# deepomicslab/PALACE

Measured on AMD Instinct MI355X. Metric: contigs/sec eref+generate_graph+matching, 1M-contig synth, 1/2/4/8 GPU, higher is better.
Workload: dtype u32

## Files before the change

include/palace_hip.h:

```cpp
#ifndef PALACE_HIP_H
#define PALACE_HIP_H

#include <stddef.h>
#include <stdint.h>

#ifdef __cplusplus
extern "C" {
#endif

#define PALACE_OK 0
#define PALACE_EINVAL (-1)
#define PALACE_EHIP (-2)
#define PALACE_ENOMEM (-3)
#define PALACE_ESTATE (-4)

typedef struct palace_ctx palace_ctx;

const char *palace_last_error(void);
const char *palace_version(void);

int palace_ctx_create(int device, palace_ctx **out);
int palace_ctx_create_prio(int device, int high_priority, palace_ctx **out);
int palace_ctx_create_on_stream(int device, void *hip_stream, palace_ctx **out);
int palace_ctx_destroy(palace_ctx *ctx);
// ... 148 lines not shown
                            int64_t n_records_total, const palace_graph_params *prm, uint64_t *d_consumed,
                            palace_graph_edge *d_edges, int64_t edge_cap, int64_t *d_n_edges, int64_t *n_edges_out);

int palace_graph_score_border(palace_ctx *ctx, palace_graph_cand *d_cands, int64_t n_cands, int64_t n_border,
                              const palace_graph_params *prm);

int palace_graph_copy_numbers(palace_ctx *ctx, const uint64_t *d_consumed, const int32_t *d_tlen,
                              int32_t n_targets, double avg_depth, int32_t *d_cn);


int palace_bgzf_inflate(palace_ctx *ctx, const uint8_t *d_in, int64_t n_members, const int64_t *d_in_off, const int32_t *d_in_len,
                        const int64_t *d_out_off, const int32_t *d_out_len, uint8_t *d_out, int32_t *d_status);


int palace_bgzf_deflate(palace_ctx *ctx, const uint8_t *d_text, int64_t n_members, const int64_t *d_off, const int32_t *d_len,
                        const uint32_t *d_crc, uint8_t *d_slots, int32_t *d_member_len);

int palace_bgzf_deflate_lz(palace_ctx *ctx, const uint8_t *d_text, int64_t n_members, const int64_t *d_off, const int32_t *d_len,
                           const uint32_t *d_crc, uint8_t *d_slots, int32_t *d_member_len);

int palace_bgzf_compact(palace_ctx *ctx, const uint8_t *d_slots, int64_t n_members, const int32_t *d_member_len, uint8_t *d_file,
                        int64_t *d_member_off);


int palace_crc32_members(palace_ctx *ctx, const uint8_t *d_data, int64_t n_members, const int64_t *d_off, const int32_t *d_len,
                         uint32_t *d_crc);

typedef struct {
    int64_t line, reads, bases;
    int32_t open, error;
} palace_fastq_cursor;

size_t palace_fastq_scratch_bytes(int64_t max_window);
int palace_fastq_parse(palace_ctx *ctx, const uint8_t *d_text, int64_t n, int final_window, palace_fastq_cursor *d_cursor,
                       uint8_t *d_bases, int64_t bases_cap, int64_t *d_offsets, int64_t offsets_cap, void *d_scratch,
                       size_t scratch_bytes);


#define PALACE_DEPTH_TAIL_BYTES 4096

typedef struct {
    int64_t lines;
    uint64_t sum;
    int64_t bad_line;
    int64_t win_runs, win_name_bytes;
    int32_t tail_len, tail_buf;
    int32_t error, reserved0;
    int64_t reserved1;
    uint8_t tail[2][PALACE_DEPTH_TAIL_BYTES];
} palace_depth_cursor;

typedef struct {
    uint64_t sum, lines;
    uint32_t name_off, name_len;
} palace_depth_run;

size_t palace_depth_parse_scratch_bytes(int64_t max_window);
int palace_depth_parse(palace_ctx *ctx, const uint8_t *d_text, int64_t n, int final_window, palace_depth_cursor *d_cursor,
                       palace_depth_run *d_runs, int64_t runs_cap, uint8_t *d_names, int64_t names_cap, void *d_scratch,
                       size_t scratch_bytes);


typedef struct {
    int64_t stride, span, text_cap;
    int64_t check_guards;
} palace_gzip_params;

enum {
    PALACE_GZ_NONE = 0,
    PALACE_GZ_HEADER = 1,
    PALACE_GZ_DECODE = 2,
    PALACE_GZ_CHAIN_OPEN = 3,
    PALACE_GZ_NO_PROGRESS = 4,
    PALACE_GZ_TOO_BIG = 5,
    PALACE_GZ_TRUNCATED = 6,
    PALACE_GZ_CRC = 7,
    PALACE_GZ_ISIZE = 8,
    PALACE_GZ_TRAILING = 9,
    PALACE_GZ_SINK = 10,
    PALACE_GZ_MARKER = 11
};

typedef struct {
    int64_t chunks_found, chunks_accepted, false_hits, rounds, members, spans, batches, text_bytes;
    int32_t fallback, guards_bad;
    double ms_upload, ms_find, ms_size, ms_decode, ms_chain, ms_resolve, ms_crc, ms_sink;
} palace_gzip_stats;

typedef int (*palace_gzip_sink)(void *user, const uint8_t *d_text, int64_t n, int last);

int palace_gzip_inflate(palace_ctx *ctx, const uint8_t *file, int64_t size, const palace_gzip_params *prm, palace_gzip_sink sink,
                        void *user, palace_gzip_stats *stats);


int palace_depth_sum_covered(palace_ctx *ctx, int64_t n_segs, const int32_t *d_seg_tid, const int32_t *d_seg_pos,
                             const int32_t *d_seg_len, int32_t n_targets, const int32_t *d_tlen, const int64_t *d_tbase,
                             int64_t total_len, uint64_t *sum_out, uint64_t *covered_out);

int palace_depth_per_contig(palace_ctx *ctx, int64_t n_segs, const int32_t *d_seg_tid, const int32_t *d_seg_pos,
                            const int32_t *d_seg_len, int32_t n_targets, const int32_t *d_tlen, const int64_t *d_tbase,
                            int64_t total_len, uint64_t *sum_out, uint64_t *covered_out, uint64_t *d_contig_sum,
                            uint64_t *d_contig_covered);

typedef struct palace_depth_text palace_depth_text;
int palace_depth_text_create(palace_ctx *ctx, int64_t n_segs, const int32_t *d_seg_tid, const int32_t *d_seg_pos,
                             const int32_t *d_seg_len, int32_t n_targets, const int32_t *d_tlen, const int64_t *d_tbase,
                             int64_t total_len, const uint8_t *d_names, const int64_t *d_name_off, palace_depth_text **out,
                             uint64_t *text_bytes_out, uint64_t *lines_out, uint64_t *sum_out);
int palace_depth_text_destroy(palace_ctx *ctx, palace_depth_text *dt);
int palace_depth_text_emit(palace_ctx *ctx, const palace_depth_text *dt, uint64_t text_begin, uint64_t text_end, uint8_t *d_out);
int palace_depth_text_windows(palace_ctx *ctx, const palace_depth_text *dt, int64_t n_windows, const int64_t *d_win_beg,
                              const int64_t *d_win_end, uint64_t *d_text_beg, uint64_t *d_text_end, uint64_t *d_lines);


size_t palace_bam_walk_scratch_bytes(int64_t total, int64_t first, int64_t chunk);
int palace_bam_walk(palace_ctx *ctx, const uint8_t *d_stream, int64_t total, int64_t first, int32_t n_ref, int64_t chunk,
                    void *d_scratch, size_t scratch_bytes, int64_t *d_starts, int64_t cap, int64_t *n_records_out,
                    int64_t *stop_out, int64_t stats_out[4]);
int palace_bam_walk_starts(palace_ctx *ctx, const uint8_t *d_stream, int64_t total, int64_t first, int64_t chunk, const void *d_scratch,
                           size_t scratch_bytes, int64_t *d_starts, int64_t cap);

int palace_bam_match_segments(palace_ctx *ctx, const uint8_t *d_stream, int64_t total, const int64_t *d_starts, int64_t n_records,
                              int32_t n_ref, int32_t *d_seg_tid, int32_t *d_seg_pos, int32_t *d_seg_len, int64_t cap,
                              int64_t *n_segs_out);


int palace_bam_columns(palace_ctx *ctx, const uint8_t *d_stream, int64_t total, const int64_t *d_starts, int64_t n_records,
                       uint64_t key_seed, const palace_bam_cols *cols);
int palace_bam_name_keys(palace_ctx *ctx, const uint8_t *d_stream, int64_t total, const int64_t *d_starts, int64_t n_records,
                         uint64_t key_seed, uint64_t *d_qkey);
int palace_bam_names_differ(palace_ctx *ctx, const uint8_t *d_stream, int64_t total, const int64_t *d_starts, int64_t n_records,
                            const int64_t *d_pairs, int64_t n_pairs, int64_t *n_differ_out);

typedef struct palace_bam_names palace_bam_names;
int palace_bam_names_create(palace_ctx *ctx, const uint8_t *d_names, const int64_t *d_name_off, int32_t n_ref, palace_bam_names **out);
int palace_bam_names_destroy(palace_ctx *ctx, palace_bam_names *names);

int palace_bam_sa_items(palace_ctx *ctx, const uint8_t *d_stream, int64_t total, const int64_t *d_starts, int64_t n_records,
                        const palace_bam_names *names, int32_t *d_sa_off, palace_sa_item *d_items, int64_t cap, int64_t *n_items_out);


int palace_match_greedy(palace_ctx *ctx, int32_t n_vertices, int64_t n_arcs, const int32_t *d_src,
                        const int32_t *d_dst, const int64_t *d_out_off, const int32_t *d_out_arcs,
                        const int64_t *d_in_off, const int32_t *d_in_arcs, const uint8_t *d_alive,
                        int32_t *d_next, int32_t *d_prev, int32_t *d_next_arc, int32_t *rounds_out);

int palace_match_arcs_from_edges(const int32_t *cn, int32_t n_segs, const palace_graph_edge *edges, int64_t n_edges,
                                 int32_t min_count, int64_t *copies, int32_t *src, int32_t *dst, int64_t *weight,
                                 int64_t *n_arcs_out);

typedef struct palace_match_result palace_match_result;
int palace_match_set_option(palace_ctx *ctx, const char *name, int64_t value);
int palace_match_last_run(palace_ctx *ctx, int64_t info[4]);
int palace_match_decompose(palace_ctx *ctx, int32_t n_segs, const int64_t *copies, int64_t n_arcs,
                           const int32_t *src, const int32_t *dst, int32_t iterations, int32_t aggressive,
                           palace_match_result **out);
int palace_match_decompose_ex(palace_ctx *ctx, int32_t n_segs, const int64_t *copies, int64_t n_arcs,
                              const int32_t *src, const int32_t *dst, int32_t iterations, int32_t aggressive,
                              int32_t compact, palace_match_result **out);
const uint64_t *palace_match_result_bare(const palace_match_result *r);
int64_t palace_match_result_bare_count(const palace_match_result *r);
int64_t palace_match_result_count(const palace_match_result *r);
const int64_t *palace_match_result_offsets(const palace_match_result *r);
const int32_t *palace_match_result_verts(const palace_match_result *r);
const uint8_t *palace_match_result_kind(const palace_match_result *r);
const int32_t *palace_match_result_iter(const palace_match_result *r);
const int32_t *palace_match_result_open_at(const palace_match_result *r);
void palace_match_result_free(palace_match_result *r);


typedef struct {
    int32_t n_segs;
    int32_t min_count;
    const uint8_t *seed;
    const int32_t *tlen;
    const int32_t *rank;
    const int32_t *name_len;
    int64_t n_paths;
    const int64_t *path_off;
    const int32_t *path_tok;
} palace_stage04_inputs;

typedef struct palace_stage04 palace_stage04;
int palace_stage04_create(palace_ctx *ctx, const palace_stage04_inputs *in, palace_stage04 **out);
int palace_stage04_destroy(palace_ctx *ctx, palace_stage04 *s);

int palace_stage04_reserve(palace_ctx *ctx, palace_stage04 *s, int64_t edge_bound);

int palace_stage04_filter(palace_ctx *ctx, palace_stage04 *s, const palace_graph_edge *d_edges, const int64_t *d_n_edges,
                          int64_t edge_bound);
int palace_stage04_flags(palace_ctx *ctx, palace_stage04 *s, uint8_t *h_seg_flags, uint8_t *h_edge_flags, int64_t n_edges);
int palace_stage04_counts(palace_ctx *ctx, palace_stage04 *s, int64_t counts[8]);

int palace_stage04_match(palace_ctx *ctx, palace_stage04 *s, const palace_graph_edge *d_edges, const int32_t *d_cn,
                         int32_t iterations, int32_t aggressive, int32_t use_paths);
int palace_stage04_result(palace_ctx *ctx, palace_stage04 *s, palace_match_result **out, const int32_t **contig_of_out,
                          int64_t *n_segs_filtered_out);


#define PALACE_FASTA_TILE_BYTES 4096

typedef struct {
    int64_t name_off, name_len, seq_off, length, line_bases, line_width;
} palace_fasta_rec;

#define PALACE_FASTA_OK 0
#define PALACE_FASTA_ETEXT 1
#define PALACE_FASTA_ENAME 2
#define PALACE_FASTA_ERAGGED 3
#define PALACE_FASTA_EBLANK 4
#define PALACE_FASTA_EBYTE 5

typedef struct {
    int64_t n_records, bad_line;
    int32_t error, reserved;
} palace_fasta_status;

size_t palace_fasta_index_scratch_bytes(int64_t n);
int palace_fasta_index(palace_ctx *ctx, const uint8_t *d_text, int64_t n, palace_fasta_rec *d_recs, int64_t recs_cap, void *d_scratch,
                       size_t scratch_bytes, palace_fasta_status *status_out);

typedef struct palace_fasta_names palace_fasta_names;
int palace_fasta_names_create(palace_ctx *ctx, const uint8_t *d_text, const palace_fasta_rec *d_recs, int64_t n_records, uint8_t *d_dup,
                              palace_fasta_names **out);
int palace_fasta_names_destroy(palace_ctx *ctx, palace_fasta_names *names);

#define PALACE_PATH_NOTHING (-1)
#define PALACE_PATH_NOT_FOUND (-2)
#define PALACE_PATH_REVERSE 1
#define PALACE_PATH_SECOND_TRY 2

int palace_path_resolve(palace_ctx *ctx, const palace_fasta_names *names, const uint8_t *d_tok, const int64_t *d_tok_off, int64_t n_tok,
                        int32_t *d_code);

int palace_path_fasta_lengths(palace_ctx *ctx, const palace_fasta_rec *d_recs, const int32_t *d_code, int64_t n_tok, const int64_t *d_path_off,
                              int64_t n_paths, int64_t *d_tok_cum, int64_t *d_path_len);

int palace_path_fasta_write(palace_ctx *ctx, const uint8_t *d_text, const palace_fasta_rec *d_recs, const int32_t *d_code,
                            const int64_t *d_tok_cum, const int64_t *d_path_off, int64_t n_paths, const uint8_t *d_hdr,
                            const int64_t *d_hdr_off, const int64_t *d_path_out, int64_t lo, int64_t hi, uint8_t *d_out);


int palace_cycle_trim(palace_ctx *ctx, const int32_t *d_node, const int32_t *d_base, const int64_t *d_len, int64_t n_tok,
                      const int64_t *d_path_off, int64_t n_paths, const uint64_t *d_arcs, int64_t n_arcs, int64_t trim_threshold,
                      int64_t min_cycle_length, int32_t *d_first, int32_t *d_last);

int palace_final_fasta_lengths(palace_ctx *ctx, const palace_fasta_rec *d_recs, const int32_t *d_code, int64_t n_tok, const int64_t *d_path_off,
                               int64_t n_paths, int64_t sep_len, int64_t *d_tok_cum, int64_t *d_path_len);

int palace_final_fasta_write(palace_ctx *ctx, const uint8_t *d_text, const palace_fasta_rec *d_recs, const int32_t *d_code,
                             const int64_t *d_tok_cum, const int64_t *d_path_off, int64_t n_paths, const uint8_t *d_hdr,
                             const int64_t *d_hdr_off, const int64_t *d_path_out, int32_t sep_byte, int64_t lo, int64_t hi, uint8_t *d_out);


#define PALACE_BLAST_ECOLUMNS 1
#define PALACE_BLAST_ENAME 2
#define PALACE_BLAST_EIDENTITY 3
#define PALACE_BLAST_ELENGTH 4
#define PALACE_BLAST_EQUERY 5
#define PALACE_BLAST_EQEMPTY 6

int palace_blast_identity_cuts(double threshold, int64_t *cut);

int palace_blast_groups(palace_ctx *ctx, const uint8_t *d_text, const int64_t *d_line_start, int64_t n_lines, const palace_fasta_names *names,
                        int64_t n_records, double blast_ratio, const int64_t *cut, uint8_t *d_seg, int64_t *out);

#define PALACE_FILTERRES_REC_GENE 1
#define PALACE_FILTERRES_REC_S07 2
#define PALACE_FILTERRES_REC_S09 4
#define PALACE_FILTERRES_REC_BLAST 8
#define PALACE_FILTERRES_TAG_SELF 1
#define PALACE_FILTERRES_TAG_CYCLE 2
#define PALACE_FILTERRES_WRITE 1
#define PALACE_FILTERRES_PLAIN 2
#define PALACE_FILTERRES_SELFGENE 4
#define PALACE_FILTERRES_CYCLEGENE 8
#define PALACE_FILTERRES_CYCLESCORE 16
#define PALACE_FILTERRES_GENESCORE 32

int palace_filter_result_plan(palace_ctx *ctx, const int32_t *d_code, const int64_t *d_path_off, int64_t n_paths, const uint8_t *d_tag,
                              const palace_fasta_rec *d_recs, const uint8_t *d_rec_bits, uint8_t *d_class, int64_t *d_all_len);

int palace_paths_first_of_equal(palace_ctx *ctx, const int32_t *d_code, const int64_t *d_path_off, int64_t n_paths, const uint8_t *d_class,
                                int32_t hash_bits, uint8_t *d_first);


#define PALACE_FASTG_EPLUS 6
#define PALACE_FASTG_EHIGH 7
#define PALACE_FASTG_ECR 8
#define PALACE_FASTG_ENOLF 9
#define PALACE_FASTG_EEMPTY 10
#define PALACE_FASTG_ENONAME 11
#define PALACE_FASTG_EBASE 12

int palace_fastg_derive(palace_ctx *ctx, const uint8_t *d_text, int64_t n, const palace_fasta_rec *d_recs, int64_t n_records,
                        palace_fasta_rec *d_name_recs, uint8_t *d_primed, palace_fasta_status *status_out);

int palace_fastg_plan(palace_ctx *ctx, const palace_fasta_rec *d_name_recs, uint8_t *d_dup, int64_t n_records, int64_t *d_out_off,
                      palace_fasta_rec *d_out_recs, int64_t *n_kept_out, int64_t *out_bytes_out);

int palace_fastg_write(palace_ctx *ctx, const uint8_t *d_text, const palace_fasta_rec *d_name_recs, const uint8_t *d_primed,
                       const int64_t *d_out_off, int64_t n_records, int64_t lo, int64_t hi, uint8_t *d_out);

int palace_fai_rows_plan(palace_ctx *ctx, const palace_fasta_rec *d_recs, const uint8_t *d_skip, int64_t n_records, int64_t *d_row_off,
                         int64_t *bytes_out);
int palace_fai_rows_write(palace_ctx *ctx, const uint8_t *d_text, const palace_fasta_rec *d_recs, const uint8_t *d_skip, int64_t n_records,
// ... 164 lines not shown
```

palace_amd/capi.py:

```python
from __future__ import annotations

import ctypes as C
import os
import subprocess

import numpy as np

_HERE = os.path.dirname(os.path.abspath(__file__))
SO_PATH = os.environ.get("PALACE_HIP_SO") or os.path.join(_HERE, "libpalace_hip.so")
_LIB = None


class PalaceError(RuntimeError):
    pass


def build(force: bool = False) -> str:
    args = ["make", "-C", os.path.join(_HERE, "csrc")]
    if force:
        subprocess.run(args + ["clean"], check=True, stdout=subprocess.DEVNULL)
    subprocess.run(args, check=True, stdout=subprocess.DEVNULL)
    return SO_PATH


# ... 2 lines not shown
                ("both_order", C.c_int32), ("reserved", C.c_int32), ("max_span_frac", C.c_double)]

    @classmethod
    def default(cls):
        return cls(300, 0, 5, 1, 0, 0, 0.80)


class BamCols(C.Structure):
    _fields_ = [("n", C.c_int64)] + [(k, C.c_void_p) for k in
                                     ("tid", "pos", "mtid", "mpos", "nm", "ref_len", "read_len", "clip_s", "clip_e",
                                      "flag", "mapq", "qkey", "sa_off")]


class GzipParams(C.Structure):
    _fields_ = [("stride", C.c_int64), ("span", C.c_int64), ("text_cap", C.c_int64), ("check_guards", C.c_int64)]


class GzipStats(C.Structure):
    _fields_ = [(k, C.c_int64) for k in ("chunks_found", "chunks_accepted", "false_hits", "rounds", "members", "spans", "batches", "text_bytes")] + \
        [("fallback", C.c_int32), ("guards_bad", C.c_int32)] + \
        [(k, C.c_double) for k in ("ms_upload", "ms_find", "ms_size", "ms_decode", "ms_chain", "ms_resolve", "ms_crc", "ms_sink")]


GZIP_SINK = C.CFUNCTYPE(C.c_int, C.c_void_p, C.c_void_p, C.c_int64, C.c_int)


class Stage04Inputs(C.Structure):
    _fields_ = [("n_segs", C.c_int32), ("min_count", C.c_int32), ("seed", C.c_void_p), ("tlen", C.c_void_p), ("rank", C.c_void_p),
                ("name_len", C.c_void_p), ("n_paths", C.c_int64), ("path_off", C.c_void_p), ("path_tok", C.c_void_p)]


SA_ITEM_DTYPE = np.dtype([(k, np.int32) for k in ("tid2", "pos2", "mapq2", "nm2", "clip_s2", "clip_e2", "len2", "rev2")])
CAND_DTYPE = np.dtype([("ord", np.int64), ("qkey", np.uint64), ("left", np.int32), ("right", np.int32),
                       ("mtid", np.int32), ("ref_len", np.int32), ("dL", np.int32), ("dR", np.int32),
                       ("nmL", np.int32), ("nmR", np.int32), ("mapqL", np.int16), ("mapqR", np.int16),
                       ("kind", np.uint8), ("cls", np.uint8), ("found", np.uint8), ("in_fastg", np.uint8),
                       ("oL", np.uint8), ("oR", np.uint8), ("pad0", np.uint8), ("pad1", np.uint8), ("sa_index", np.int32)])
EDGE_DTYPE = np.dtype([("left", np.int32), ("right", np.int32), ("counts", np.uint32, 4), ("oL", np.uint8),
                       ("oR", np.uint8), ("pad", np.uint8, 6)])
FASTQ_CURSOR_DTYPE = np.dtype([("line", np.int64), ("reads", np.int64), ("bases", np.int64), ("open", np.int32), ("error", np.int32)])
DEPTH_CURSOR_DTYPE = np.dtype([("lines", np.int64), ("sum", np.uint64), ("bad_line", np.int64), ("win_runs", np.int64), ("win_name_bytes", np.int64),
                               ("tail_len", np.int32), ("tail_buf", np.int32), ("error", np.int32), ("reserved0", np.int32), ("reserved1", np.int64),
                               ("tail", np.uint8, (2, 4096))])
DEPTH_RUN_DTYPE = np.dtype([("sum", np.uint64), ("lines", np.uint64), ("name_off", np.uint32), ("name_len", np.uint32)])
assert DEPTH_CURSOR_DTYPE.itemsize == 64 + 8192 and DEPTH_RUN_DTYPE.itemsize == 24
FASTA_REC_DTYPE = np.dtype([(k, np.int64) for k in ("name_off", "name_len", "seq_off", "length", "line_bases", "line_width")])
FASTA_TILE_BYTES = 4096
FAIDX_REGION_DTYPE = np.dtype([(k, np.int64) for k in ("rec", "beg", "len")])
CONTIG_FEATURES, CONTIG_FSUMS, CONTIG_CHUNK_BASES = 12288, 64, 4096
CONTIG_INFO_DTYPE = np.dtype([("length", np.int64), ("bases", np.int64)])
PATH_NOTHING, PATH_NOT_FOUND, PATH_REVERSE, PATH_SECOND_TRY = -1, -2, 1, 2


class BaiStatus(C.Structure):
    _fields_ = [("n_bad", C.c_int64), ("first_bad", C.c_int64), ("first_unsorted", C.c_int64), ("n_no_coor", C.c_int64)]


SORT_TILE = 4096


class FastaStatus(C.Structure):
    _fields_ = [("n_records", C.c_int64), ("bad_line", C.c_int64), ("error", C.c_int32), ("reserved", C.c_int32)]


class ReadqcParams(C.Structure):
    _fields_ = [(k, C.c_int32) for k in ("qualified_quality", "unqualified_percent", "n_limit", "min_length", "no_trim", "no_quality_filter",
                                         "no_length_filter", "overlap_require", "diff_limit", "diff_pct", "diff_window", "reserved")]

    @classmethod
    def default(cls, **kw):
        p = cls(15, 40, 5, 15, 0, 0, 0, 30, 5, 20, 50, 0)
        for k, v in kw.items():
            assert hasattr(p, k), k
            setattr(p, k, int(v))
        return p


READQC_OUT = ("reads_before", "bases_before", "reads_after", "bases_after", "low_quality", "too_many_n", "too_short", "trimmed_reads", "trimmed_bases",
              "bytes_1", "bytes_2")
READQC_ISIZE_MAX = 512
READQC_CYCLE_TILE = 256

assert CAND_DTYPE.itemsize == 64 and EDGE_DTYPE.itemsize == 32 and SA_ITEM_DTYPE.itemsize == 32 and C.sizeof(ReadqcParams) == 48

_SIGS = {
    "palace_ctx_create": [C.c_int, C.POINTER(C.c_void_p)],
    "palace_ctx_create_prio": [C.c_int, C.c_int, C.POINTER(C.c_void_p)],
    "palace_ctx_create_on_stream": [C.c_int, C.c_void_p, C.POINTER(C.c_void_p)],
    "palace_ctx_destroy": [C.c_void_p],
    "palace_sync": [C.c_void_p],
    "palace_malloc": [C.c_void_p, C.c_size_t, C.POINTER(C.c_void_p)],
    "palace_free": [C.c_void_p, C.c_void_p],
    "palace_memset": [C.c_void_p, C.c_void_p, C.c_int, C.c_size_t],
    "palace_h2d": [C.c_void_p, C.c_void_p, C.c_void_p, C.c_size_t],
    "palace_d2h": [C.c_void_p, C.c_void_p, C.c_void_p, C.c_size_t],
    "palace_d2d": [C.c_void_p, C.c_void_p, C.c_void_p, C.c_size_t],
    "palace_host_alloc": [C.c_void_p, C.c_size_t, C.POINTER(C.c_void_p)],
    "palace_host_free": [C.c_void_p, C.c_void_p],
    "palace_d2h_async": [C.c_void_p, C.c_void_p, C.c_void_p, C.c_size_t],
    "palace_h2d_async": [C.c_void_p, C.c_void_p, C.c_void_p, C.c_size_t],
    "palace_mark_wait": [C.c_void_p, C.c_int],
    "palace_mark_wait_for": [C.c_void_p, C.c_int, C.c_double],
    "palace_wait_for_mark": [C.c_void_p, C.c_void_p, C.c_int],
    "palace_timer_begin": [C.c_void_p],
    "palace_timer_end": [C.c_void_p, C.POINTER(C.c_float)],
    "palace_mark": [C.c_void_p, C.c_int],
    "palace_mark_elapsed": [C.c_void_p, C.c_int, C.c_int, C.POINTER(C.c_float)],
    "palace_eref_set_coder": [C.c_void_p, C.c_void_p],
    "palace_eref_index_refs": [C.c_void_p, C.c_void_p, C.c_void_p, C.c_int64, C.c_void_p, C.c_void_p],
    "palace_eref_table_reset": [C.c_void_p],
    "palace_eref_reserve": [C.c_void_p, C.c_int64],
    "palace_eref_count_reads": [C.c_void_p, C.c_void_p, C.c_void_p, C.c_int64, C.c_void_p, C.c_int64],
    "palace_eref_pack_reads": [C.c_void_p, C.c_void_p, C.c_void_p, C.c_int64, C.c_void_p, C.c_int64, C.c_void_p, C.c_void_p, C.c_void_p],
    "palace_eref_count_reads_packed": [C.c_void_p, C.c_void_p, C.c_void_p, C.c_void_p, C.c_int64, C.c_int64],
    "palace_eref_set_count_mode": [C.c_void_p, C.c_int, C.c_int64],
    "palace_eref_set_key_buckets": [C.c_void_p, C.c_void_p],
    "palace_eref_set_option": [C.c_void_p, C.c_char_p, C.c_int64],
    "palace_eref_scan_refs": [C.c_void_p, C.c_void_p, C.c_void_p, C.c_int64, C.c_int64, C.c_int, C.c_int,
                              C.c_void_p],
    "palace_eref_probe_index_build": [C.c_void_p, C.c_void_p, C.c_void_p, C.c_int64, C.c_int64, C.POINTER(C.c_void_p)],
    "palace_eref_attach_probe_index": [C.c_void_p, C.c_void_p],
    "palace_eref_entry_layout": [C.c_void_p, C.POINTER(C.c_size_t), C.POINTER(C.c_size_t)],
    "palace_eref_entry_buffers_attach": [C.c_void_p, C.c_void_p, C.c_void_p, C.c_void_p],
    "palace_eref_entry_buffers": [C.c_void_p, C.POINTER(C.c_void_p), C.POINTER(C.c_void_p)],
    "palace_eref_entry_hits_from_counts": [C.c_void_p, C.c_void_p, C.c_void_p, C.c_int, C.c_size_t, C.c_size_t, C.c_size_t],
    "palace_eref_entry_hits_complete": [C.c_void_p, C.c_void_p, C.c_int64],
    "palace_eref_entry_counts_valid": [C.c_void_p, C.c_void_p],
    "palace_eref_probe_index_free": [C.c_void_p, C.c_void_p],
    "palace_eref_scan_refs_indexed": [C.c_void_p, C.c_void_p, C.c_void_p, C.c_void_p, C.c_int64, C.c_int64, C.c_int, C.c_int,
                                      C.c_void_p],
    "palace_eref_table_planes": [C.c_void_p, C.POINTER(C.c_void_p), C.POINTER(C.c_size_t)],
    "palace_eref_table_attach": [C.c_void_p, C.POINTER(C.c_void_p)],
    "palace_eref_table_invalidate": [C.c_void_p],
    "palace_eref_table_merge_slices": [C.c_void_p, C.c_void_p, C.c_int, C.c_size_t, C.c_size_t],
    "palace_eref_table_merge_slices_packed": [C.c_void_p, C.c_void_p, C.c_int, C.c_size_t, C.c_size_t],
    "palace_eref_table_pack_low": [C.c_void_p, C.c_void_p],
    "palace_eref_plane_pack": [C.c_void_p, C.c_void_p, C.c_void_p, C.c_void_p, C.c_int64, C.c_void_p],
    "palace_eref_plane_unpack": [C.c_void_p, C.c_void_p, C.c_void_p, C.c_void_p, C.c_int64, C.c_void_p],
    "palace_eref_table_lookup": [C.c_void_p, C.c_void_p, C.c_int64, C.c_void_p],
    "palace_eref_table_popcounts": [C.c_void_p, C.POINTER(C.c_uint64)],
    "palace_graph_classify": [C.c_void_p, C.POINTER(BamCols), C.c_void_p, C.c_int32, C.c_void_p, C.c_void_p,
                              C.c_void_p, C.c_int64, C.POINTER(GraphParams), C.c_int64, C.c_void_p, C.c_void_p,
                              C.c_int64, C.POINTER(C.c_int64)],
    "palace_depth_sum_covered": [C.c_void_p, C.c_int64, C.c_void_p, C.c_void_p, C.c_void_p, C.c_int32, C.c_void_p, C.c_void_p, C.c_int64,
                                 C.POINTER(C.c_uint64), C.POINTER(C.c_uint64)],
    "palace_depth_per_contig": [C.c_void_p, C.c_int64, C.c_void_p, C.c_void_p, C.c_void_p, C.c_int32, C.c_void_p, C.c_void_p, C.c_int64,
                                C.POINTER(C.c_uint64), C.POINTER(C.c_uint64), C.c_void_p, C.c_void_p],
    "palace_graph_copy_numbers": [C.c_void_p, C.c_void_p, C.c_void_p, C.c_int32, C.c_double, C.c_void_p],
    "palace_match_greedy": [C.c_void_p, C.c_int32, C.c_int64] + [C.c_void_p] * 10 + [C.POINTER(C.c_int32)],
    "palace_match_arcs_from_edges": [C.c_void_p, C.c_int32, C.c_void_p, C.c_int64, C.c_int32, C.c_void_p, C.c_void_p,
                                     C.c_void_p, C.c_void_p, C.POINTER(C.c_int64)],
    "palace_match_set_option": [C.c_void_p, C.c_char_p, C.c_int64],
    "palace_match_last_run": [C.c_void_p, C.POINTER(C.c_int64)],
    "palace_match_decompose":[C.c_void_p, C.c_int32, C.c_void_p, C.c_int64, C.c_void_p, C.c_void_p, C.c_int32,
                               C.c_int32, C.POINTER(C.c_void_p)],
    "palace_match_decompose_ex": [C.c_void_p, C.c_int32, C.c_void_p, C.c_int64, C.c_void_p, C.c_void_p, C.c_int32,
                                  C.c_int32, C.c_int32, C.POINTER(C.c_void_p)],
    "palace_graph_resolve": [C.c_void_p, C.c_void_p, C.c_int64, C.c_int64, C.POINTER(GraphParams), C.c_void_p,
                             C.c_void_p, C.c_int64, C.POINTER(C.c_int64)],
    "palace_graph_classify_ex": [C.c_void_p, C.POINTER(BamCols), C.c_void_p, C.c_int32, C.c_void_p, C.c_void_p,
                                 C.c_void_p, C.c_int64, C.POINTER(GraphParams), C.c_int64, C.c_void_p, C.c_void_p,
                                 C.c_int64, C.POINTER(C.c_int64), C.POINTER(C.c_int64)],
    "palace_graph_classify_ix": [C.c_void_p, C.POINTER(BamCols), C.c_void_p, C.c_int32, C.c_void_p, C.c_void_p,
                                 C.c_void_p, C.c_int64, C.c_void_p, C.POINTER(GraphParams), C.c_int64, C.c_void_p, C.c_void_p,
                                 C.c_int64, C.POINTER(C.c_int64), C.POINTER(C.c_int64)],
    "palace_graph_fastg_offsets": [C.c_void_p, C.c_void_p, C.c_int64, C.c_int32, C.c_void_p],
    "palace_bgzf_inflate": [C.c_void_p, C.c_void_p, C.c_int64, C.c_void_p, C.c_void_p, C.c_void_p, C.c_void_p, C.c_void_p, C.c_void_p],
    "palace_fastq_scratch_bytes": [C.c_int64],
    "palace_crc32_members": [C.c_void_p, C.c_void_p, C.c_int64, C.c_void_p, C.c_void_p, C.c_void_p],
    "palace_bgzf_deflate": [C.c_void_p, C.c_void_p, C.c_int64, C.c_void_p, C.c_void_p, C.c_void_p, C.c_void_p, C.c_void_p],
    "palace_bgzf_deflate_lz": [C.c_void_p, C.c_void_p, C.c_int64, C.c_void_p, C.c_void_p, C.c_void_p, C.c_void_p, C.c_void_p],
    "palace_bgzf_compact": [C.c_void_p, C.c_void_p, C.c_int64, C.c_void_p, C.c_void_p, C.c_void_p],
    "palace_depth_text_create": [C.c_void_p, C.c_int64, C.c_void_p, C.c_void_p, C.c_void_p, C.c_int32, C.c_void_p, C.c_void_p, C.c_int64,
                                 C.c_void_p, C.c_void_p, C.POINTER(C.c_void_p), C.POINTER(C.c_uint64), C.POINTER(C.c_uint64), C.POINTER(C.c_uint64)],
    "palace_depth_text_destroy": [C.c_void_p, C.c_void_p],
    "palace_depth_text_emit": [C.c_void_p, C.c_void_p, C.c_uint64, C.c_uint64, C.c_void_p],
    "palace_depth_text_windows": [C.c_void_p, C.c_void_p, C.c_int64, C.c_void_p, C.c_void_p, C.c_void_p, C.c_void_p, C.c_void_p],
    "palace_gzip_inflate": [C.c_void_p, C.c_void_p, C.c_int64, C.POINTER(GzipParams), GZIP_SINK, C.c_void_p, C.POINTER(GzipStats)],
    "palace_fastq_parse": [C.c_void_p, C.c_void_p, C.c_int64, C.c_int, C.c_void_p, C.c_void_p, C.c_int64, C.c_void_p, C.c_int64,
                           C.c_void_p, C.c_size_t],
    "palace_depth_parse_scratch_bytes": [C.c_int64],
    "palace_depth_parse": [C.c_void_p, C.c_void_p, C.c_int64, C.c_int, C.c_void_p, C.c_void_p, C.c_int64, C.c_void_p, C.c_int64,
                           C.c_void_p, C.c_size_t],
    "palace_graph_score_border": [C.c_void_p, C.c_void_p, C.c_int64, C.c_int64, C.POINTER(GraphParams)],
    "palace_graph_resolve_ex": [C.c_void_p, C.c_void_p, C.c_int64, C.c_int64, C.c_int64, C.POINTER(GraphParams), C.c_void_p,
                                C.c_void_p, C.c_int64, C.c_void_p, C.POINTER(C.c_int64)],
    "palace_bam_walk_scratch_bytes": [C.c_int64, C.c_int64, C.c_int64],
    "palace_bam_walk": [C.c_void_p, C.c_void_p, C.c_int64, C.c_int64, C.c_int32, C.c_int64, C.c_void_p, C.c_size_t, C.c_void_p, C.c_int64,
                        C.POINTER(C.c_int64), C.POINTER(C.c_int64), C.POINTER(C.c_int64)],
    "palace_bam_walk_starts": [C.c_void_p, C.c_void_p, C.c_int64, C.c_int64, C.c_int64, C.c_void_p, C.c_size_t, C.c_void_p, C.c_int64],
    "palace_bam_match_segments": [C.c_void_p, C.c_void_p, C.c_int64, C.c_void_p, C.c_int64, C.c_int32, C.c_void_p, C.c_void_p, C.c_void_p,
                                  C.c_int64, C.POINTER(C.c_int64)],
    "palace_bam_columns": [C.c_void_p, C.c_void_p, C.c_int64, C.c_void_p, C.c_int64, C.c_uint64, C.POINTER(BamCols)],
    "palace_bam_name_keys": [C.c_void_p, C.c_void_p, C.c_int64, C.c_void_p, C.c_int64, C.c_uint64, C.c_void_p],
    "palace_bam_names_differ": [C.c_void_p, C.c_void_p, C.c_int64, C.c_void_p, C.c_int64, C.c_void_p, C.c_int64, C.POINTER(C.c_int64)],
    "palace_bam_names_create": [C.c_void_p, C.c_void_p, C.c_void_p, C.c_int32, C.POINTER(C.c_void_p)],
    "palace_bam_names_destroy": [C.c_void_p, C.c_void_p],
    "palace_bam_sa_items": [C.c_void_p, C.c_void_p, C.c_int64, C.c_void_p, C.c_int64, C.c_void_p, C.c_void_p, C.c_void_p, C.c_int64,
                            C.POINTER(C.c_int64)],
    "palace_stage04_create": [C.c_void_p, C.POINTER(Stage04Inputs), C.POINTER(C.c_void_p)],
    "palace_stage04_destroy": [C.c_void_p, C.c_void_p],
    "palace_stage04_reserve": [C.c_void_p, C.c_void_p, C.c_int64],
    "palace_stage04_filter": [C.c_void_p, C.c_void_p, C.c_void_p, C.c_void_p, C.c_int64],
    "palace_stage04_flags": [C.c_void_p, C.c_void_p, C.c_void_p, C.c_void_p, C.c_int64],
    "palace_stage04_counts": [C.c_void_p, C.c_void_p, C.POINTER(C.c_int64)],
    "palace_stage04_match": [C.c_void_p, C.c_void_p, C.c_void_p, C.c_void_p, C.c_int32, C.c_int32, C.c_int32],
    "palace_stage04_result": [C.c_void_p, C.c_void_p, C.POINTER(C.c_void_p), C.POINTER(C.c_void_p), C.POINTER(C.c_int64)],
    "palace_fasta_index_scratch_bytes": [C.c_int64],
    "palace_fasta_index": [C.c_void_p, C.c_void_p, C.c_int64, C.c_void_p, C.c_int64, C.c_void_p, C.c_size_t, C.POINTER(FastaStatus)],
    "palace_fasta_names_create": [C.c_void_p, C.c_void_p, C.c_void_p, C.c_int64, C.c_void_p, C.POINTER(C.c_void_p)],
    "palace_fasta_names_destroy": [C.c_void_p, C.c_void_p],
    "palace_path_resolve": [C.c_void_p, C.c_void_p, C.c_void_p, C.c_void_p, C.c_int64, C.c_void_p],
    "palace_path_fasta_lengths": [C.c_void_p, C.c_void_p, C.c_void_p, C.c_int64, C.c_void_p, C.c_int64, C.c_void_p, C.c_void_p],
    "palace_fastg_derive": [C.c_void_p, C.c_void_p, C.c_int64, C.c_void_p, C.c_int64, C.c_void_p, C.c_void_p, C.POINTER(FastaStatus)],
    "palace_fastg_plan": [C.c_void_p, C.c_void_p, C.c_void_p, C.c_int64, C.c_void_p, C.c_void_p, C.POINTER(C.c_int64), C.POINTER(C.c_int64)],
    "palace_fastg_write": [C.c_void_p, C.c_void_p, C.c_void_p, C.c_void_p, C.c_void_p, C.c_int64, C.c_int64, C.c_int64, C.c_void_p],
    "palace_fai_rows_plan": [C.c_void_p, C.c_void_p, C.c_void_p, C.c_int64, C.c_void_p, C.POINTER(C.c_int64)],
    "palace_fai_rows_write": [C.c_void_p, C.c_void_p, C.c_void_p, C.c_void_p, C.c_int64, C.c_void_p, C.c_void_p],
    "palace_faidx_resolve": [C.c_void_p, C.c_void_p, C.c_void_p, C.c_void_p, C.c_void_p, C.c_int64, C.c_void_p],
    "palace_faidx_plan": [C.c_void_p, C.c_void_p, C.c_int64, C.c_void_p, C.c_int64, C.c_int, C.c_void_p, C.POINTER(C.c_int64), C.POINTER(C.c_int64)],
    "palace_faidx_write": [C.c_void_p, C.c_void_p, C.c_void_p, C.c_void_p, C.c_int64, C.c_void_p, C.c_void_p, C.c_void_p, C.c_int64, C.c_int, C.c_int64,
                           C.c_int64, C.c_void_p],
    "palace_path_fasta_write": [C.c_void_p, C.c_void_p, C.c_void_p, C.c_void_p, C.c_void_p, C.c_void_p, C.c_int64, C.c_void_p, C.c_void_p,
                                C.c_void_p, C.c_int64, C.c_int64, C.c_void_p],
    "palace_cycle_trim": [C.c_void_p, C.c_void_p, C.c_void_p, C.c_void_p, C.c_int64, C.c_void_p, C.c_int64, C.c_void_p, C.c_int64, C.c_int64, C.c_int64,
                          C.c_void_p, C.c_void_p],
    "palace_final_fasta_lengths": [C.c_void_p, C.c_void_p, C.c_void_p, C.c_int64, C.c_void_p, C.c_int64, C.c_int64, C.c_void_p, C.c_void_p],
    "palace_final_fasta_write": [C.c_void_p, C.c_void_p, C.c_void_p, C.c_void_p, C.c_void_p, C.c_void_p, C.c_int64, C.c_void_p, C.c_void_p,
                                 C.c_void_p, C.c_int32, C.c_int64, C.c_int64, C.c_void_p],
    "palace_blast_identity_cuts": [C.c_double, C.POINTER(C.c_int64)],
    "palace_blast_groups": [C.c_void_p, C.c_void_p, C.c_void_p, C.c_int64, C.c_void_p, C.c_int64, C.c_double, C.POINTER(C.c_int64), C.c_void_p,
                            C.POINTER(C.c_int64)],
    "palace_filter_result_plan": [C.c_void_p, C.c_void_p, C.c_void_p, C.c_int64, C.c_void_p, C.c_void_p, C.c_void_p, C.c_void_p, C.c_void_p],
    "palace_paths_first_of_equal": [C.c_void_p, C.c_void_p, C.c_void_p, C.c_int64, C.c_void_p, C.c_int32, C.c_void_p],
    "palace_bam_sort_keys": [C.c_void_p, C.c_void_p, C.c_int64, C.c_void_p, C.c_int64, C.c_int32, C.c_void_p, C.POINTER(C.c_int64), C.POINTER(C.c_int64)],
    "palace_sort_u64_scratch_bytes": [C.c_int64],
    "palace_sort_u64": [C.c_void_p, C.c_void_p, C.c_void_p, C.c_int64, C.c_int32, C.c_void_p, C.c_size_t],
    "palace_bam_gather_plan": [C.c_void_p, C.c_void_p, C.c_void_p, C.c_void_p, C.c_int64, C.c_int64, C.c_void_p, C.c_void_p, C.POINTER(C.c_int64)],
    "palace_bam_gather_write": [C.c_void_p, C.c_void_p, C.c_void_p, C.c_void_p, C.c_void_p, C.c_int64, C.c_int64, C.c_void_p],
    "palace_bai_records": [C.c_void_p, C.c_void_p, C.c_void_p, C.c_int64, C.c_int32, C.c_void_p, C.c_void_p, C.c_void_p, C.c_void_p, C.c_void_p,
                           C.POINTER(BaiStatus)],
    "palace_bai_chunks": [C.c_void_p, C.c_void_p, C.c_void_p, C.c_void_p, C.c_void_p, C.c_int64, C.c_int32, C.c_void_p, C.c_void_p, C.c_void_p, C.c_void_p,
                          C.c_int64, C.POINTER(C.c_int64)],
    "palace_bai_linear": [C.c_void_p, C.c_void_p, C.c_void_p, C.c_void_p, C.c_void_p, C.c_void_p, C.c_void_p, C.c_int64, C.c_int32, C.c_void_p, C.c_void_p,
                          C.c_void_p, C.c_int64, C.c_void_p],
    "palace_bgzf_voffsets": [C.c_void_p, C.c_void_p, C.c_int64, C.c_void_p, C.c_void_p, C.c_int64, C.c_void_p],
    "palace_sam_scratch_bytes": [C.c_int64],
    "palace_sam_lines": [C.c_void_p, C.c_void_p, C.c_int64, C.c_void_p, C.c_size_t, C.c_void_p, C.c_int64, C.POINTER(C.c_int64)],
    "palace_sam_plan": [C.c_void_p, C.c_void_p, C.c_void_p, C.c_int64, C.c_int64, C.c_void_p, C.c_uint32, C.c_int64, C.c_void_p, C.c_void_p, C.c_void_p,
                        C.POINTER(C.c_int64)],
    "palace_sam_encode": [C.c_void_p, C.c_void_p, C.c_void_p, C.c_int64, C.c_void_p, C.c_void_p, C.c_void_p, C.c_void_p, C.c_void_p, C.c_void_p],
    "palace_fastq_records": [C.c_void_p, C.c_void_p, C.c_void_p, C.c_int64, C.c_void_p, C.POINTER(C.c_int64)],
    "palace_readqc_plan": [C.c_void_p, C.c_void_p, C.c_void_p, C.c_void_p, C.c_void_p, C.c_int64, C.POINTER(ReadqcParams), C.c_void_p, C.c_void_p, C.c_void_p,
                           C.c_void_p, C.POINTER(C.c_int64)],
    "palace_readqc_write": [C.c_void_p, C.c_void_p, C.c_void_p, C.c_void_p, C.c_void_p, C.c_int64, C.c_int64, C.c_int64, C.c_void_p],
    "palace_readqc_plan_ex": [C.c_void_p, C.c_void_p, C.c_void_p, C.c_void_p, C.c_void_p, C.c_int64, C.POINTER(ReadqcParams), C.c_void_p, C.c_void_p, C.c_void_p,
                              C.c_void_p, C.c_void_p, C.POINTER(C.c_int64)],
    "palace_readqc_insert_sizes": [C.c_void_p, C.c_void_p, C.c_void_p, C.c_void_p, C.c_int64, C.POINTER(ReadqcParams), C.c_void_p],
    "palace_readqc_cycle_stats": [C.c_void_p, C.c_void_p, C.c_void_p, C.c_int64, C.c_void_p, C.c_int32, C.c_void_p],
    "palace_contig_features_scratch_bytes": [C.c_int64, C.c_int64],
    "palace_contig_features": [C.c_void_p, C.c_void_p, C.c_int64, C.c_void_p, C.c_int64, C.c_int64, C.c_void_p, C.c_void_p, C.c_void_p, C.c_void_p,
                               C.c_void_p, C.c_size_t],
}


def declared_symbols():
    import re
    text = open(os.path.join(_HERE, "..", "include", "palace_hip.h")).read()
    text = re.sub(r"/\*.*?\*/", "", text, flags=re.S)
    return sorted(set(re.findall(r"\b(palace_[a-z0-9_]+)\s*\(", text)))


def lib() -> C.CDLL:
    global _LIB
    if _LIB is None:
        if not os.path.exists(SO_PATH):
            raise PalaceError(f"{SO_PATH} is missing: run `python -c 'import __graft_entry__ as g; g.build()'` "
                              "(hipcc --offload-arch=gfx950). There is no CPU fallback.")
        _LIB = C.CDLL(SO_PATH)
        _LIB.palace_last_error.restype = C.c_char_p
        _LIB.palace_version.restype = C.c_char_p
        _LIB.palace_stream.restype = C.c_void_p
        _LIB.palace_stream.argtypes = [C.c_void_p]
        _LIB.palace_eref_packed_bytes.restype = C.c_size_t
        _LIB.palace_eref_packed_bytes.argtypes = [C.c_int64]
        for nm, rt in (("count", C.c_int64), ("bare_count", C.c_int64), ("bare", C.POINTER(C.c_uint64)), ("offsets", C.POINTER(C.c_int64)), ("verts", C.POINTER(C.c_int32)),
                       ("kind", C.POINTER(C.c_uint8)), ("iter", C.POINTER(C.c_int32)), ("open_at", C.POINTER(C.c_int32))):
            fn = getattr(_LIB, "palace_match_result_" + nm)
            fn.argtypes = [C.c_void_p]
            fn.restype = rt
        _LIB.palace_match_result_free.argtypes = [C.c_void_p]
        _LIB.palace_match_result_free.restype = None
        for name, sig in _SIGS.items():
            fn = getattr(_LIB, name)
            fn.argtypes = sig
            fn.restype = C.c_int
        _LIB.palace_fastq_scratch_bytes.restype = C.c_size_t
        _LIB.palace_bam_walk_scratch_bytes.restype = C.c_size_t
        _LIB.palace_depth_parse_scratch_bytes.restype = C.c_size_t
        _LIB.palace_fasta_index_scratch_bytes.restype = C.c_size_t
        _LIB.palace_sort_u64_scratch_bytes.restype = C.c_size_t
        _LIB.palace_sam_scratch_bytes.restype = C.c_size_t
        _LIB.palace_contig_features_scratch_bytes.restype = C.c_size_t
    return _LIB


# ... 955 lines not shown

    def close(self):
        for b in self.bufs:
            b.free()
        self.bufs = []


BAM_COLUMNS = (("tid", np.int32), ("pos", np.int32), ("mtid", np.int32), ("mpos", np.int32), ("nm", np.int32), ("ref_len", np.int32),
               ("read_len", np.int32), ("clip_s", np.int32), ("clip_e", np.int32), ("flag", np.uint16), ("mapq", np.uint8), ("qkey", np.uint64))


def bam_decode(ctx: Ctx, stream: bytes, starts, names, key_seed: int = 1):
    stream = bytes(stream)
    st = np.ascontiguousarray(starts, dtype=np.int64)
    n = len(st)
    blob = b"".join(names)
    off = np.zeros(len(names) + 1, np.int64)
    off[1:] = np.cumsum([len(x) for x in names])
    bufs = [ctx.upload(np.frombuffer(stream, dtype=np.uint8) if stream else np.zeros(1, np.uint8)), ctx.upload(st if n else np.zeros(1, np.int64)),
            ctx.upload(np.frombuffer(blob, dtype=np.uint8) if blob else np.zeros(1, np.uint8)), ctx.upload(off)]
    d_stream, d_st, d_blob, d_off = bufs
    table = C.c_void_p()
    try:
        col = {k: ctx.empty(max(1, n), dt) for k, dt in BAM_COLUMNS}
        col["sa_off"] = ctx.empty(n + 1, np.int32)
        bufs += list(col.values())
        cols = BamCols(n, **{k: b.ptr for k, b in col.items()})
        _check(lib().palace_bam_columns(ctx.h, d_stream.ptr, len(stream), d_st.ptr, n, key_seed, C.byref(cols)), "palace_bam_columns")
        _check(lib().palace_bam_names_create(ctx.h, d_blob.ptr, d_off.ptr, len(names), C.byref(table)), "palace_bam_names_create")
        cnt = C.c_int64()
        _check(lib().palace_bam_sa_items(ctx.h, d_stream.ptr, len(stream), d_st.ptr, n, table, None, None, 0, C.byref(cnt)), "palace_bam_sa_items")
        want = cnt.value
        d_items = ctx.empty(max(1, want), SA_ITEM_DTYPE)
        bufs.append(d_items)
        _check(lib().palace_bam_sa_items(ctx.h, d_stream.ptr, len(stream), d_st.ptr, n, table, col["sa_off"].ptr, d_items.ptr, want, C.byref(cnt)),
               "palace_bam_sa_items")
        assert cnt.value == want
        out = {k: b.to_host()[:n + 1 if k == "sa_off" else n].copy() for k, b in col.items()}
        return out, d_items.to_host()[:want].copy()
    finally:
        if table:
            lib().palace_bam_names_destroy(ctx.h, table)
        for b in bufs:
            b.free()


def bam_name_keys(ctx: Ctx, stream: bytes, starts, key_seed: int):
    stream = bytes(stream)
    st = np.ascontiguousarray(starts, dtype=np.int64)
    bufs = [ctx.upload(np.frombuffer(stream, dtype=np.uint8)), ctx.upload(st), ctx.empty(max(1, len(st)), np.uint64)]
    try:
        _check(lib().palace_bam_name_keys(ctx.h, bufs[0].ptr, len(stream), bufs[1].ptr, len(st), key_seed, bufs[2].ptr), "palace_bam_name_keys")
        return bufs[2].to_host()[:len(st)].copy()
    finally:
        for b in bufs:
            b.free()


def bam_names_differ(ctx: Ctx, stream: bytes, starts, pairs) -> int:
    stream = bytes(stream)
    st = np.ascontiguousarray(starts, dtype=np.int64)
    pr = np.ascontiguousarray(pairs, dtype=np.int64).reshape(-1, 2)
    bufs = [ctx.upload(np.frombuffer(stream, dtype=np.uint8)), ctx.upload(st), ctx.upload(pr if len(pr) else np.zeros((1, 2), np.int64))]
    n = C.c_int64()
    try:
        _check(lib().palace_bam_names_differ(ctx.h, bufs[0].ptr, len(stream), bufs[1].ptr, len(st), bufs[2].ptr, len(pr), C.byref(n)),
               "palace_bam_names_differ")
        return int(n.value)
    finally:
        for b in bufs:
            b.free()


_ARC_BUFFERS = {}


def match_arcs_from_edges(cn: np.ndarray, edges: np.ndarray, min_count: int = 5, reuse: bool = False):
    cn = np.ascontiguousarray(cn, dtype=np.int32)
    e = np.ascontiguousarray(edges, dtype=EDGE_DTYPE)
    key = (len(cn), len(e))
    if reuse and key in _ARC_BUFFERS:
        copies, src, dst, w = _ARC_BUFFERS[key]
    else:
        copies = np.empty(len(cn), np.int64)
        src = np.empty(2 * len(e), np.int32); dst = np.empty(2 * len(e), np.int32); w = np.empty(2 * len(e), np.int64)
        if reuse:
            _ARC_BUFFERS.clear()
            _ARC_BUFFERS[key] = (copies, src, dst, w)
    n = C.c_int64()
    _check(lib().palace_match_arcs_from_edges(cn.ctypes.data, len(cn), e.ctypes.data, len(e), min_count, copies.ctypes.data,
                                              src.ctypes.data, dst.ctypes.data, w.ctypes.data, C.byref(n)),
           "palace_match_arcs_from_edges")
    return copies, src[:n.value], dst[:n.value], w[:n.value]


class MatchResult:

    def __init__(self, handle):
        L = lib()
        self._h = handle
        n = self.n = L.palace_match_result_count(handle)
        self.off = np.ctypeslib.as_array(L.palace_match_result_offsets(handle), shape=(n + 1,))
        nv = int(self.off[-1])
        self.verts = np.ctypeslib.as_array(L.palace_match_result_verts(handle), shape=(max(nv, 1),))[:nv]
        mk = lambda f, dt: (np.ctypeslib.as_array(f(handle), shape=(max(n, 1),))[:n] if n else np.zeros(0, dt))
        self.kind = mk(L.palace_match_result_kind, np.uint8)
        self.iter = mk(L.palace_match_result_iter, np.int32)
        self.open_at = mk(L.palace_match_result_open_at, np.int32)

    def free(self):
        if self._h is not None:
            self.off = self.verts = self.kind = self.iter = self.open_at = None
            lib().palace_match_result_free(self._h)
            self._h = None

    def __enter__(self):
        return self

    def __exit__(self, *exc):
        self.free()


def match_decompose_views(ctx: "Ctx", copies: np.ndarray, src: np.ndarray, dst: np.ndarray, iterations: int = 10,
                          aggressive: bool = False, compact: bool = False) -> MatchResult:
    cp = np.ascontiguousarray(copies, dtype=np.int64)
    s = np.ascontiguousarray(src, dtype=np.int32)
    d = np.ascontiguousarray(dst, dtype=np.int32)
    res = C.c_void_p()
    _check(lib().palace_match_decompose_ex(ctx.h, len(cp), cp.ctypes.data, len(s), s.ctypes.data, d.ctypes.data,
                                           iterations, int(aggressive), int(compact), C.byref(res)), "palace_match_decompose")
    r = MatchResult(res)
    if compact:
        r.n_bare = int(lib().palace_match_result_bare_count(res))
        words = (len(cp) + 63) // 64
        r.bare = np.ctypeslib.as_array(lib().palace_match_result_bare(res), shape=(max(1, words),))[:words]
    return r


def match_decompose(ctx: "Ctx", copies: np.ndarray, src: np.ndarray, dst: np.ndarray, iterations: int = 10,
                    aggressive: bool = False):
    with match_decompose_views(ctx, copies, src, dst, iterations, aggressive) as r:
        return r.off.copy(), r.verts.copy(), r.kind.copy(), r.iter.copy(), r.open_at.copy()


MATCH_KEYS_POSITION, MATCH_KEYS_TWO_WORDS, MATCH_KEYS_ONE_WORD = 0, 1, 2


def match_last_run(ctx: "Ctx") -> dict:
    info = (C.c_int64 * 4)()
    _check(lib().palace_match_last_run(ctx.h, info), "palace_match_last_run")
    return dict(key_mode=int(info[0]), checked_rerun=bool(info[1]), rounds=int(info[2]), iterations=int(info[3]))


def match_greedy(ctx: "Ctx", n_vertices: int, src, dst, alive=None):
    s = np.ascontiguousarray(src, dtype=np.int32)
    d = np.ascontiguousarray(dst, dtype=np.int32)
    al = np.ones(n_vertices, np.uint8) if alive is None else np.ascontiguousarray(alive, dtype=np.uint8)
    assert len(s) == len(d) and len(al) == n_vertices
    assert not len(s) or (0 <= min(s.min(), d.min()) and max(s.max(), d.max()) < n_vertices)

    def csr(ends):
        off = np.zeros(n_vertices + 1, np.int64)
        np.cumsum(np.bincount(ends, minlength=n_vertices), out=off[1:])
        return off, np.argsort(ends, kind="stable").astype(np.int32)

    (out_off, out_arcs), (in_off, in_arcs) = csr(s), csr(d)
    bufs = [ctx.upload(a) for a in (s, d, out_off, out_arcs, in_off, in_arcs, al)]
    outs = [ctx.empty(max(1, n_vertices), np.int32) for _ in range(3)]
    rounds = C.c_int32()
    try:
        _check(lib().palace_match_greedy(ctx.h, n_vertices, len(s), *(b.ptr for b in bufs), *(o.ptr for o in outs), C.byref(rounds)),
               "palace_match_greedy")
        nxt, prv, arc = (o.to_host()[:n_vertices] for o in outs)
    finally:
        for b in bufs + outs:
            b.free()
    return nxt, prv, arc, rounds.value


class Stage04:
    COUNT_NAMES = ("edges", "juncs", "kept_pass2", "kept_pass3_more", "segs_selected", "segs_rescued", "arcs", "segs_filtered")

    def __init__(self, ctx: "Ctx", seed, tlen, rank, name_len, path_off, path_tok, min_count: int = 5):
        self.ctx = ctx
        self._keep = [np.ascontiguousarray(seed, np.uint8), np.ascontiguousarray(tlen, np.int32), np.ascontiguousarray(rank, np.int32),
                      np.ascontiguousarray(name_len, np.int32), np.ascontiguousarray(path_off, np.int64),
                      np.ascontiguousarray(path_tok, np.int32)]
        sd, tl, rk, nl, po, pt = self._keep
        assert len(sd) == len(tl) == len(rk) == len(nl) and len(po) >= 1
        inp = Stage04Inputs(len(sd), min_count, sd.ctypes.data, tl.ctypes.data, rk.ctypes.data, nl.ctypes.data, len(po) - 1,
                            po.ctypes.data, pt.ctypes.data if len(pt) else None)
        h = C.c_void_p()
        _check(lib().palace_stage04_create(ctx.h, C.byref(inp), C.byref(h)), "palace_stage04_create")
        self.h, self.n_segs = h, len(sd)

    def filter(self, d_edges_ptr: int, d_n_edges_ptr: int, edge_bound: int):
        _check(lib().palace_stage04_filter(self.ctx.h, self.h, d_edges_ptr, d_n_edges_ptr, edge_bound), "palace_stage04_filter")

    def counts(self) -> dict:
        out = (C.c_int64 * 8)()
        _check(lib().palace_stage04_counts(self.ctx.h, self.h, out), "palace_stage04_counts")
        return dict(zip(self.COUNT_NAMES, (int(v) for v in out)))

    def flags(self, n_edges: int):
        seg = np.zeros(self.n_segs, np.uint8)
        edge = np.zeros(n_edges, np.uint8)
        _check(lib().palace_stage04_flags(self.ctx.h, self.h, seg.ctypes.data, edge.ctypes.data if n_edges else None, n_edges),
               "palace_stage04_flags")
        return seg, edge

    def match(self, d_edges_ptr: int, d_cn_ptr: int, iterations: int = 10, aggressive: bool = False, use_paths: bool = True):
        _check(lib().palace_stage04_match(self.ctx.h, self.h, d_edges_ptr, d_cn_ptr, iterations, int(aggressive), int(use_paths)), "palace_stage04_match")

    def result(self):
        res, cof, n = C.c_void_p(), C.c_void_p(), C.c_int64()
        _check(lib().palace_stage04_result(self.ctx.h, self.h, C.byref(res), C.byref(cof), C.byref(n)), "palace_stage04_result")
        r = MatchResult(res)
        r.n_bare = int(lib().palace_match_result_bare_count(res))
        words = (n.value + 63) // 64
        r.bare = np.ctypeslib.as_array(lib().palace_match_result_bare(res), shape=(max(1, words),))[:words]
        contig_of = np.ctypeslib.as_array(C.cast(cof, C.POINTER(C.c_int32)), shape=(max(1, n.value),))[: n.value]
        return r, contig_of

    def close(self):
        if self.h:
            lib().palace_stage04_destroy(self.ctx.h, self.h)
            self.h = None


def window_minimums(hit_ratio: float, perfect_ratio: float):
    w = np.float32(500)
    return int(w * np.float32(hit_ratio)), int(w * np.float32(perfect_ratio))


def fasta_index(ctx: Ctx, text: bytes, recs_cap: int | None = None):
    a = np.frombuffer(text, dtype=np.uint8)
    d_text = ctx.upload(a)
    d_scratch = DevBuf(ctx, max(int(lib().palace_fasta_index_scratch_bytes(len(a))), 1))
    st = FastaStatus()
    if recs_cap is None:
        _check(lib().palace_fasta_index(ctx.h, d_text.ptr, len(a), None, 0, d_scratch.ptr, d_scratch.nbytes, C.byref(st)), "palace_fasta_index")
        recs_cap = int(st.n_records)
    d_recs = ctx.empty((max(recs_cap, 1),), FASTA_REC_DTYPE)
    _check(lib().palace_fasta_index(ctx.h, d_text.ptr, len(a), d_recs.ptr, recs_cap, d_scratch.ptr, d_scratch.nbytes, C.byref(st)), "palace_fasta_index")
    d_scratch.free()
    recs = d_recs.to_host()[:int(st.n_records)] if int(st.n_records) <= recs_cap else None
    return st, recs, d_text, d_recs


def fasta_index_at(ctx: Ctx, text_ptr: int, n: int, recs_ptr, recs_cap: int, scratch_ptr: int, scratch_bytes: int) -> FastaStatus:
    st = FastaStatus()
    _check(lib().palace_fasta_index(ctx.h, text_ptr, n, recs_ptr, recs_cap, scratch_ptr, scratch_bytes, C.byref(st)), "palace_fasta_index")
    return st


def contig_features_enqueue(ctx: Ctx, text_ptr: int, n: int, recs_ptr: int, r0: int, r1: int, feat_ptr: int, fsum_ptr: int, info_ptr, bad_ptr: int,
                            scratch_ptr: int, scratch_bytes: int):
    _check(lib().palace_contig_features(ctx.h, text_ptr, n, recs_ptr, r0, r1, feat_ptr, fsum_ptr, info_ptr, bad_ptr, scratch_ptr, scratch_bytes),
           "palace_contig_features")


def contig_features(ctx: Ctx, text: bytes, r0: int = 0, r1: int | None = None, guard_rows: int = 1, repeat: int = 1):
    st, recs, d_text, d_recs = fasta_index(ctx, text)
    if st.error:
        return st, recs, None, None, None, None
    n_rec = int(st.n_records)
    r1 = n_rec if r1 is None else r1
    rows = r1 - r0
    outs = []
    for width, dtype in ((CONTIG_FEATURES, np.float32), (CONTIG_FSUMS, np.float32), (1, CONTIG_INFO_DTYPE)):
        outs.append(ctx.upload(np.full((rows + 2 * guard_rows) * width * np.dtype(dtype).itemsize, 0xA5, np.uint8)))
    d_bad = ctx.upload(np.array([12345], np.int64))
    need = int(lib().palace_contig_features_scratch_bytes(len(text), rows))
    d_scratch = DevBuf(ctx, max(need, 1))
    at = [b.ptr + guard_rows * w * isz for b, w, isz in zip(outs, (CONTIG_FEATURES, CONTIG_FSUMS, 1), (4, 4, 16))]
    for _ in range(repeat):
        contig_features_enqueue(ctx, d_text.ptr, len(text), d_recs.ptr, r0, r1, at[0], at[1], at[2], d_bad.ptr, d_scratch.ptr, need)
    ctx.sync()
    got = []
    for b, width, dtype in zip(outs, (CONTIG_FEATURES, CONTIG_FSUMS, 1), (np.float32, np.float32, CONTIG_INFO_DTYPE)):
        raw = b.to_host()
        g = guard_rows * width * np.dtype(dtype).itemsize
        if not ((raw[:g] == 0xA5).all() and (raw[len(raw) - g:] == 0xA5).all()):
            raise PalaceError("palace_contig_features wrote outside its rows")
        got.append(raw[g:len(raw) - g].view(dtype).reshape(rows, width) if width > 1 else raw[g:len(raw) - g].view(dtype))
    bad = int(d_bad.to_host()[0])
    for b in outs + [d_bad, d_scratch, d_text, d_recs]:
        b.free()
    return st, recs, got[0], got[1], got[2], bad


class PathFasta:

    def __init__(self, ctx: Ctx, text: bytes):
        self.ctx = ctx
        self.status, self.recs, self.d_text, self.d_recs = fasta_index(ctx, text)
        assert self.status.error == 0, (self.status.error, self.status.bad_line)
        self.n = int(self.status.n_records)
        self.d_dup = ctx.empty((max(self.n, 1),), np.uint8)
        self.names = C.c_void_p()
        _check(lib().palace_fasta_names_create(ctx.h, self.d_text.ptr, self.d_recs.ptr, self.n, self.d_dup.ptr, C.byref(self.names)), "palace_fasta_names_create")

    def duplicates(self) -> np.ndarray:
        return self.d_dup.to_host()[:self.n]

    def resolve(self, tokens):
# ... 312 lines not shown
```

palace_amd/csrc/common.hpp:

```cpp
#pragma once
#include <hip/hip_runtime.h>
#include <cstdarg>
#include <cstdint>
#include <cstdio>
#include <cstring>
#include <vector>

#include "../../include/palace_hip.h"
#include "eref_table_state.hpp"

namespace palace {

void set_error(const char *fmt, ...);

#define PALACE_HIP_TRY(expr)                                                                    \
    do {                                                                                        \
        hipError_t e__ = (expr);                                                                \
        if (e__ != hipSuccess) {                                                                \
            palace::set_error("%s failed: %s (%s:%d)", #expr, hipGetErrorString(e__), __FILE__, \
                              __LINE__);                                                        \
            return PALACE_EHIP;                                                                 \
        }                                                                                       \
    } while (0)

#define PALACE_REQUIRE_AS(name, cond, msg)                         \
    do {                                                           \
        if (!(cond)) {                                             \
            palace::set_error("%s: %s", name, msg);                \
            return PALACE_EINVAL;                                  \
        }                                                          \
    } while (0)
#define PALACE_REQUIRE(cond, msg) PALACE_REQUIRE_AS(__func__, cond, msg)

constexpr int kWave = 64;
constexpr int kCUs = 256;
constexpr size_t kPlaneBytes = 1ull << 29;
constexpr size_t kPlaneWords = 1ull << 27;

struct CoderMasks {
    uint32_t m[3][3];
};

inline size_t align256(size_t b) { return (b + 255) & ~static_cast<size_t>(255); }

struct Workspace {
    void *ptr = nullptr;
    size_t bytes = 0;
};

}

namespace palace {
struct MatchScratch;
void free_match_scratch(MatchScratch *m);
}

struct palace_ctx {
    int device = 0;
    hipStream_t stream = nullptr;
    bool owns_stream = true;
    hipEvent_t ev0 = nullptr, ev1 = nullptr;
    uint32_t key_buckets[4] = {~0u, ~0u, ~0u, ~0u};
    std::vector<hipEvent_t> marks;
    bool coder_set = false;
    palace::CoderMasks masks{};
    uint32_t *plane[3] = {nullptr, nullptr, nullptr};
    bool planes_external = false;
    palace::TableState table;
    bool want_final = false;
    const struct palace_eref_probe_index *probe_ix = nullptr;
    int probe_all_sets = 0;
    int64_t scan_ref_lo = 0, scan_ref_hi = 0;
    int count_mode = 0;
    int64_t bin_cap_override = 0;
    int64_t slab_override = 0;
    palace::Workspace ws;
    bool ws_grown = false;
    palace::Workspace pin;
    palace::MatchScratch *match_scratch = nullptr;
    int64_t graph_border = -1;
    const void *graph_border_cands = nullptr;
    int64_t graph_border_n = -1;
    int match_grid = 0;
    bool match_two_word_keys = false;
    int match_iters = 0;
    int64_t match_last[4] = {-1, 0, 0, 0};
    uint64_t *d_small = nullptr;
};

namespace palace {
int ensure_workspace(palace_ctx *ctx, size_t bytes);
int ensure_pinned(palace_ctx *ctx, size_t bytes);
int ensure_table(palace_ctx *ctx);
}
```

palace_amd/csrc/decomp.hip:

```cpp
#include "decomp.hpp"

#include <algorithm>

namespace palace {

namespace {

constexpr uint64_t kNoKey = ~0ull;
constexpr uint64_t kClosed = 0;
constexpr int kStampShift = 42;
constexpr int kPackedShift = 52, kPackedStamps = 1 << (64 - kPackedShift);
constexpr uint64_t kLenMask = (1ull << 40) - 1;


__device__ __forceinline__ uint64_t wave_incl_scan(uint64_t v, int lane)
{
#pragma unroll
    for (int d = 1; d < 64; d <<= 1) {
        const uint64_t u = __shfl_up(v, d);
        if (lane >= d) v += u;
    }
    return v;
}

constexpr int kMaxWaves = 16;

__device__ void scan_partials_body(const uint64_t *__restrict__ in, int64_t n, uint64_t *__restrict__ partials, int blk, int nblk)
{
    __shared__ uint64_t part[kMaxWaves];
    const int64_t chunk = (n + nblk - 1) / nblk;
    const int64_t a = min(n, static_cast<int64_t>(blk) * chunk), e = min(n, a + chunk);
    uint64_t s = 0;
    for (int64_t i = a + threadIdx.x; i < e; i += blockDim.x) s += in[i];
    const int lane = threadIdx.x & 63, waves = static_cast<int>(blockDim.x >> 6);
    s = wave_incl_scan(s, lane);
    if (lane == 63) part[threadIdx.x >> 6] = s;
    __syncthreads();
    if (threadIdx.x == 0) {
        uint64_t t = 0;
        for (int w = 0; w < waves; w++) t += part[w];
        partials[blk] = t;
    }
    __syncthreads();
}

__device__ void scan_prefix_body(uint64_t *__restrict__ partials, int n_parts, uint64_t *__restrict__ total)
{
    __shared__ uint64_t part[kMaxWaves];
    const int lane = threadIdx.x & 63, wv = threadIdx.x >> 6;
    const uint64_t x = static_cast<int>(threadIdx.x) < n_parts ? partials[threadIdx.x] : 0;
    const uint64_t incl = wave_incl_scan(x, lane);
    if (lane == 63) part[wv] = incl;
    __syncthreads();
    uint64_t before = 0;
    for (int w = 0; w < wv; w++) before += part[w];
    if (static_cast<int>(threadIdx.x) < n_parts) partials[threadIdx.x] = before + incl - x;
    if (threadIdx.x == blockDim.x - 1) *total = before + incl;
    __syncthreads();
}

__device__ void scan_apply_body(const uint64_t *__restrict__ in, uint64_t *__restrict__ out, int64_t n, const uint64_t *__restrict__ partials,
                                int blk, int nblk)
{
    __shared__ uint64_t part[kMaxWaves];
    const int64_t chunk = (n + nblk - 1) / nblk;
    const int64_t a = min(n, static_cast<int64_t>(blk) * chunk), e = min(n, a + chunk);
    const int lane = threadIdx.x & 63, wv = threadIdx.x >> 6, waves = static_cast<int>(blockDim.x >> 6);
    uint64_t carry = partials[blk];
    for (int64_t base = a; base < e; base += blockDim.x) {
        const int64_t i = base + threadIdx.x;
        const uint64_t x = i < e ? in[i] : 0;
        const uint64_t incl = wave_incl_scan(x, lane);
        if (lane == 63) part[wv] = incl;
        __syncthreads();
        uint64_t before = 0, all = 0;
        for (int w = 0; w < waves; w++) { if (w < wv) before += part[w]; all += part[w]; }
        if (i < e) out[i] = carry + before + incl - x;
        carry += all;
        __syncthreads();
    }
}

__global__ __launch_bounds__(kDecompBlock) void scan_partials_kernel(const uint64_t *__restrict__ in, const int32_t *__restrict__ n_dev,
                                                                     uint64_t *__restrict__ partials)
{
    scan_partials_body(in, *n_dev, partials, static_cast<int>(blockIdx.x), static_cast<int>(gridDim.x));
}
__global__ __launch_bounds__(kDecompBlock) void scan_prefix_kernel(uint64_t *__restrict__ partials, int n_parts, uint64_t *__restrict__ total)
{
    scan_prefix_body(partials, n_parts, total);
}
__global__ __launch_bounds__(kDecompBlock) void scan_apply_kernel(const uint64_t *__restrict__ in, uint64_t *__restrict__ out,
                                                                  const int32_t *__restrict__ n_dev, const uint64_t *__restrict__ partials)
{
    scan_apply_body(in, out, *n_dev, partials, static_cast<int>(blockIdx.x), static_cast<int>(gridDim.x));
}

struct Span { int tid, n; };
__device__ __forceinline__ Span whole_grid() { return Span{static_cast<int>(blockIdx.x * blockDim.x + threadIdx.x), static_cast<int>(gridDim.x * blockDim.x)}; }

__device__ void ph_init(const DecompBufs &b, Span T, int64_t comp_cap, int64_t vert_cap, int n_flags, int allow_packed)
{
    DecompState *st = b.st;
    const int V = st->V;
    for (int i = T.tid; i < V; i += T.n) { b.bo_hi[i] = kNoKey; b.bi_hi[i] = kNoKey; b.on_path[i] = 0; }
    for (int i = T.tid; i < n_flags; i += T.n) b.changed[i] = 0;
    if (T.tid == 0) {
        st->n_comp = 0; st->n_vert = 0; st->comp_cap = comp_cap; st->vert_cap = vert_cap;
        st->unsettled = 0; st->overflow = 0; st->bad = 0; st->dead = 0; st->scan_total = 0; st->alive_after = 0;
        st->packed = (allow_packed && b.kc && b.pack_bad && *b.pack_bad == 0) ? 1u : 0u;
        if (comp_cap >= 0) b.o_off[0] = 0;
    }
}

__device__ void ph_round_begin(const DecompBufs &b, Span T, int reset_left)
{
    const int V = b.st->V;
    if (!reset_left && b.st->dead) return;
    if (T.tid == 0) { b.st->alive_after = 0; if (reset_left) b.st->dead = 0; }
    const int64_t E = b.st->E;
    for (int64_t e = T.tid; e < E; e += T.n) b.done[e] = 0;
    const bool packed = b.st->packed != 0;
    for (int i = T.tid; i < V; i += T.n) {
        const int s = i >> 1;
        const int64_t l = reset_left ? 1 : b.left[s];
        if (reset_left && !(i & 1)) b.left[s] = 1;
        b.alive[i] = l > 0;
        b.next[i] = -1; b.prev[i] = -1;
        b.bo_hi[i] = b.bi_hi[i] = l > 0 ? kNoKey : kClosed;
        if (!packed) { b.bo_lo[i] = kNoKey; b.bo_lo[V + i] = kNoKey; b.bi_lo[i] = kNoKey; b.bi_lo[V + i] = kNoKey; }
        b.len_a[i] = 0;
    }
}

struct IterArgs {
    uint64_t stamp;
    uint64_t stamp_p;
    int parity;
    int prev_flag, flag;
    int unique_hi;
};


__device__ void ph_propose_hi(const DecompBufs &b, Span T, const IterArgs &a)
{
    if (b.st->dead) return;
    if (a.prev_flag >= 0 && !b.changed[a.prev_flag]) return;
    const int64_t E = b.st->E;
    const int V = b.st->V;
    const int other = (a.parity ^ 1) * V;
    const bool packed = b.st->packed != 0;
    for (int64_t e = T.tid; e < E; e += T.n) {
        if (b.done[e]) continue;
        const int u = b.src[e], v = b.dst[e];
        if (b.bi_hi[v] == kClosed) { b.done[e] = 1; continue; }
        const uint64_t k = packed ? (a.stamp_p | b.kc[e]) : (a.stamp | b.khi[e]);
        if (atomicMin(reinterpret_cast<unsigned long long *>(&b.bo_hi[u]), static_cast<unsigned long long>(k)) == kClosed) { b.done[e] = 1; continue; }
        atomicMin(reinterpret_cast<unsigned long long *>(&b.bi_hi[v]), static_cast<unsigned long long>(k));
        if (!a.unique_hi && !packed) { b.bo_lo[other + u] = kNoKey; b.bi_lo[other + v] = kNoKey; }
    }
}

__device__ void ph_propose_lo(const DecompBufs &b, Span T, const IterArgs &a)
{
    if (b.st->dead) return;
    if (a.prev_flag >= 0 && !b.changed[a.prev_flag]) return;
    if (b.st->packed) return;
    const int64_t E = b.st->E;
    const int mine = a.parity * b.st->V;
    for (int64_t e = T.tid; e < E; e += T.n) {
        if (b.done[e]) continue;
        const int u = b.src[e], v = b.dst[e];
        const uint64_t k = a.stamp | b.khi[e], lo = b.klo[e];
        if (b.bo_hi[u] == k) atomicMin(reinterpret_cast<unsigned long long *>(&b.bo_lo[mine + u]), static_cast<unsigned long long>(lo));
        if (b.bi_hi[v] == k) atomicMin(reinterpret_cast<unsigned long long *>(&b.bi_lo[mine + v]), static_cast<unsigned long long>(lo));
    }
}

__device__ void ph_commit_flag(const DecompBufs &b, Span T, const IterArgs &a, volatile unsigned int *took);
__device__ void ph_commit(const DecompBufs &b, Span T, const IterArgs &a)
{
    if (b.st->dead) return;
    if (a.prev_flag >= 0 && !b.changed[a.prev_flag]) return;
    ph_commit_flag(b, T, a, b.changed + a.flag);
}
__device__ void ph_commit_flag(const DecompBufs &b, Span T, const IterArgs &a, volatile unsigned int *took)
{
    bool any = false;
    const int64_t E = b.st->E;
    const int mine = a.parity * b.st->V;
    const bool packed = b.st->packed != 0;
    for (int64_t e = T.tid; e < E; e += T.n) {
        if (b.done[e]) continue;
        const int u = b.src[e], v = b.dst[e];
        const uint64_t k = packed ? (a.stamp_p | b.kc[e]) : (a.stamp | b.khi[e]);
        if (b.bo_hi[u] != k || b.bi_hi[v] != k) continue;
        const uint64_t lo = b.klo[e];
        if (!a.unique_hi && !packed && (b.bo_lo[mine + u] != lo || b.bi_lo[mine + v] != lo)) continue;
        b.next[u] = v; b.prev[v] = u;
        b.nhi[u] = b.khi[e]; b.nlo[u] = lo;
        b.bo_hi[u] = kClosed; b.bi_hi[v] = kClosed;
        b.done[e] = 1;
        any = true;
    }
    if (__syncthreads_or(any) && threadIdx.x == 0) *took = 1u;
}

__device__ void ph_heads(const DecompBufs &b, Span T, int round, int last_flag)
{
    DecompState *st = b.st;
    if (st->dead) return;
    if (T.tid == 0 && last_flag >= 0 && b.changed[last_flag]) st->unsettled = 1;
    const int V = st->V;
    for (int v = T.tid; v < V; v += T.n) {
        if (!b.alive[v] || b.prev[v] >= 0) continue;
        int len = 0, last = v;
        int64_t least = b.left[v >> 1];
        for (int x = v; x >= 0; x = b.next[x]) {
            b.on_path[x] = round + 1;
            last = x;
            len++;
            least = min(least, b.left[x >> 1]);
        }
        const int twin_first = last ^ 1;
        if (v > twin_first) continue;
        const int64_t uses = twin_first == v ? 2 : 1;
        b.len_a[v] = (1ull << 40) | static_cast<uint64_t>(len);
        b.pay[v] = max(static_cast<int64_t>(1), least / uses);
        b.kind[v] = 0;
        b.open_at[v] = 0;
    }
}

__device__ void ph_cycles(const DecompBufs &b, Span T, int round)
{
    const int V = b.st->V;
    if (b.st->dead) return;
    for (int v = T.tid; v < V; v += T.n) {
        if (!b.alive[v] || b.on_path[v] == round + 1) continue;
        int len = 1, twin_least = v ^ 1, worst = 0;
        uint64_t whi = b.nhi[v], wlo = b.nlo[v];
        int64_t least = b.left[v >> 1];
        bool first = true;
        for (int x = b.next[v]; x != v; x = b.next[x]) {
            if (x < v) { first = false; break; }
            twin_least = min(twin_least, x ^ 1);
            const uint64_t hi = b.nhi[x], lo = b.nlo[x];
            if (hi > whi || (hi == whi && lo > wlo)) { whi = hi; wlo = lo; worst = len; }
            least = min(least, b.left[x >> 1]);
            len++;
        }
        if (!first || v > twin_least) continue;
        const int64_t uses = twin_least == v ? 2 : 1;
        b.len_a[v] = (1ull << 40) | static_cast<uint64_t>(len);
        b.pay[v] = max(static_cast<int64_t>(1), least / uses);
        b.kind[v] = 1;
        b.open_at[v] = (worst + 1) % len;
    }
}

__device__ void ph_emit(const DecompBufs &b, Span T, int round, int64_t c0, int64_t v0)
{
    DecompState *st = b.st;
    const int V = st->V;
    if (st->dead) return;
    int64_t alive = 0;
    for (int v = T.tid; v < V; v += T.n) {
        const uint64_t la = b.len_a[v];
        if (!la) continue;
        const int64_t len = static_cast<int64_t>(la & kLenMask);
        const uint64_t p = b.pos[v];
        const int64_t c = c0 + static_cast<int64_t>(p >> 40), at = v0 + static_cast<int64_t>(p & kLenMask);
        const int64_t pay = b.pay[v];
        const bool room = c < st->comp_cap && at + len <= st->vert_cap;
        if (!room) st->overflow = 1;
        else { b.o_off[c] = at; b.o_kind[c] = b.kind[v]; b.o_iter[c] = round; b.o_open[c] = b.open_at[v]; }
        int x = v;
        int64_t still = 0;
        for (int64_t k = 0; k < len; k++) {
            if (room) b.o_verts[at + k] = 2 * b.orig[x >> 1] + (x & 1);
            const int64_t l = b.left[x >> 1];
            b.left[x >> 1] = max(static_cast<int64_t>(0), l - pay);
            still += l - pay > 0;
            x = b.next[x];
        }
        alive += still;
    }
    __shared__ unsigned long long wg_alive;
    if (threadIdx.x == 0) wg_alive = 0;
    __syncthreads();
    if (alive) atomicAdd(&wg_alive, static_cast<unsigned long long>(alive));
    __syncthreads();
    if (threadIdx.x == 0 && wg_alive) atomicAdd(reinterpret_cast<unsigned long long *>(&st->alive_after), wg_alive);
}


__global__ void dec_init_kernel(DecompBufs b, int64_t comp_cap, int64_t vert_cap, int n_flags, int allow_packed) { ph_init(b, whole_grid(), comp_cap, vert_cap, n_flags, allow_packed); }
__global__ void dec_round_begin_kernel(DecompBufs b, int reset_left) { ph_round_begin(b, whole_grid(), reset_left); }
__global__ void dec_propose_hi_kernel(DecompBufs b, IterArgs a) { ph_propose_hi(b, whole_grid(), a); }
__global__ void dec_propose_lo_kernel(DecompBufs b, IterArgs a) { ph_propose_lo(b, whole_grid(), a); }
__global__ void dec_commit_kernel(DecompBufs b, IterArgs a) { ph_commit(b, whole_grid(), a); }
__global__ void dec_heads_kernel(DecompBufs b, int round, int last_flag) { ph_heads(b, whole_grid(), round, last_flag); }
__global__ void dec_cycles_kernel(DecompBufs b, int round) { ph_cycles(b, whole_grid(), round); }
__global__ void dec_emit_kernel(DecompBufs b, int round) { ph_emit(b, whole_grid(), round, b.st->n_comp, b.st->n_vert); }

__global__ void dec_round_end_kernel(DecompBufs b)
{
    DecompState *st = b.st;
    if (blockIdx.x || threadIdx.x || st->dead) return;
    st->dead = st->alive_after == 0;
    st->n_comp += static_cast<int64_t>(st->scan_total >> 40);
    st->n_vert += static_cast<int64_t>(st->scan_total & kLenMask);
    if (st->n_comp <= st->comp_cap) b.o_off[st->n_comp] = st->n_vert;
}

size_t up256(size_t v) { return (v + 255) / 256 * 256; }

struct Carver {
    char *base;
    size_t used = 0;
    template <class T>
    T *take(size_t n)
    {
        T *p = base ? reinterpret_cast<T *>(base + used) : nullptr;
        used += up256(std::max<size_t>(1, n) * sizeof(T));
        return p;
    }
};

size_t carve_all(DecompBufs &b, char *base, int64_t s_cap, int64_t e_cap, int64_t comp_cap, int64_t vert_cap, int rounds, int iters)
{
    Carver c{base};
    const size_t S = static_cast<size_t>(std::max<int64_t>(1, s_cap)), V = 2 * S, E = static_cast<size_t>(std::max<int64_t>(1, e_cap));
    b.st = c.take<DecompState>(1);
    b.src = c.take<int32_t>(E); b.dst = c.take<int32_t>(E);
    b.khi = c.take<uint64_t>(E); b.klo = c.take<uint64_t>(E);
    b.done = c.take<uint8_t>(E);
    b.kc = c.take<uint64_t>(E);
    b.left = c.take<int64_t>(S); b.orig = c.take<int32_t>(S);
    b.next = c.take<int32_t>(V); b.prev = c.take<int32_t>(V); b.on_path = c.take<int32_t>(V); b.open_at = c.take<int32_t>(V);
    b.nhi = c.take<uint64_t>(V); b.nlo = c.take<uint64_t>(V);
    b.bo_hi = c.take<uint64_t>(V); b.bi_hi = c.take<uint64_t>(V);
    b.bo_lo = c.take<uint64_t>(2 * V); b.bi_lo = c.take<uint64_t>(2 * V);
    b.len_a = c.take<uint64_t>(V); b.pos = c.take<uint64_t>(V);
    b.pay = c.take<int64_t>(V);
    b.alive = c.take<uint8_t>(V); b.kind = c.take<uint8_t>(V);
    b.partials = c.take<uint64_t>(kDecompGrid + 1);
    b.changed = c.take<uint32_t>(static_cast<size_t>(rounds) * static_cast<size_t>(iters));
    b.o_off = c.take<int64_t>(static_cast<size_t>(comp_cap) + 1);
    b.o_verts = c.take<int32_t>(static_cast<size_t>(vert_cap));
    b.o_iter = c.take<int32_t>(static_cast<size_t>(comp_cap));
    b.o_open = c.take<int32_t>(static_cast<size_t>(comp_cap));
    b.o_kind = c.take<uint8_t>(static_cast<size_t>(comp_cap));
    return c.used;
}

}

size_t decomp_bytes(int64_t s_cap, int64_t e_cap, int64_t comp_cap, int64_t vert_cap, int rounds, int iters)
{
    DecompBufs tmp;
    return carve_all(tmp, nullptr, s_cap, e_cap, comp_cap, vert_cap, rounds, iters);
}

void decomp_carve(DecompBufs &b, char *base, int64_t s_cap, int64_t e_cap, int64_t comp_cap, int64_t vert_cap, int rounds, int iters)
{
    carve_all(b, base, s_cap, e_cap, comp_cap, vert_cap, rounds, iters);
}

int scan_u64(palace_ctx *ctx, const uint64_t *in, uint64_t *out, const int32_t *n_dev, uint64_t *partials, uint64_t *total_dev)
{
    hipLaunchKernelGGL(scan_partials_kernel, dim3(kDecompGrid), dim3(kDecompBlock), 0, ctx->stream, in, n_dev, partials);
    hipLaunchKernelGGL(scan_prefix_kernel, dim3(1), dim3(kDecompBlock), 0, ctx->stream, partials, kDecompGrid, total_dev);
    hipLaunchKernelGGL(scan_apply_kernel, dim3(kDecompGrid), dim3(kDecompBlock), 0, ctx->stream, in, out, n_dev, partials);
    PALACE_HIP_TRY(hipGetLastError());
    return PALACE_OK;
}

namespace {

const dim3 kBlock(kDecompBlock);
constexpr int kWideGridDefault = 2048;
inline dim3 wide_grid(const palace_ctx *ctx) { return dim3(ctx->match_grid > 0 ? ctx->match_grid : kWideGridDefault); }

void enqueue_iterations(palace_ctx *ctx, const DecompBufs &b, int first, int n, uint64_t *count, int flag0, bool unique_hi)
{
    for (int k = 0; k < n; k++) {
        IterArgs a{((1ull << 21) - 1 - *count) << kStampShift, static_cast<uint64_t>((kPackedStamps - 1 - *count) & (kPackedStamps - 1)) << kPackedShift,
                   (first + k) & 1, k ? flag0 + k - 1 : -1, flag0 + k, unique_hi ? 1 : 0};
        (*count)++;
        hipLaunchKernelGGL(dec_propose_hi_kernel, wide_grid(ctx), kBlock, 0, ctx->stream, b, a);
        if (!unique_hi) hipLaunchKernelGGL(dec_propose_lo_kernel, wide_grid(ctx), kBlock, 0, ctx->stream, b, a);
        hipLaunchKernelGGL(dec_commit_kernel, wide_grid(ctx), kBlock, 0, ctx->stream, b, a);
    }
}

int enqueue_read_off(palace_ctx *ctx, const DecompBufs &b, int round, int last_flag)
{
    hipLaunchKernelGGL(dec_heads_kernel, wide_grid(ctx), kBlock, 0, ctx->stream, b, round, last_flag);
    hipLaunchKernelGGL(dec_cycles_kernel, wide_grid(ctx), kBlock, 0, ctx->stream, b, round);
    int rc = scan_u64(ctx, b.len_a, b.pos, &b.st->V, b.partials, &b.st->scan_total);
    if (rc) return rc;
    hipLaunchKernelGGL(dec_emit_kernel, wide_grid(ctx), kBlock, 0, ctx->stream, b, round);
    hipLaunchKernelGGL(dec_round_end_kernel, dim3(1), dim3(64), 0, ctx->stream, b);
    PALACE_HIP_TRY(hipGetLastError());
    return PALACE_OK;
}

}

int decomp_begin(palace_ctx *ctx, const DecompBufs &b, int rounds, int64_t comp_cap, int64_t vert_cap)
{
    PALACE_REQUIRE(rounds >= 1 && rounds <= kMaxRounds, "round count out of range");
    static_assert(kDecompGrid <= kDecompBlock, "scan_prefix_kernel scans the block sums with one workgroup");
    const int allow_packed = !ctx->match_two_word_keys && static_cast<int64_t>(rounds) * kMaxIters < kPackedStamps ? 1 : 0;
    hipLaunchKernelGGL(dec_init_kernel, wide_grid(ctx), kBlock, 0, ctx->stream, b, comp_cap, vert_cap, rounds * kMaxIters, allow_packed);
    PALACE_HIP_TRY(hipGetLastError());
    return PALACE_OK;
}

int decomp_rounds(palace_ctx *ctx, const DecompBufs &b, int t0, int t1, int rounds, int aggressive, int iters, bool unique_hi,
                  uint64_t *count)
{
    PALACE_REQUIRE(0 <= t0 && t0 <= t1 && t1 <= rounds && rounds <= kMaxRounds && iters >= 1 && iters <= kMaxIters, "round / iteration count out of range");
    for (int t = t0; t < t1; t++) {
        hipLaunchKernelGGL(dec_round_begin_kernel, wide_grid(ctx), kBlock, 0, ctx->stream, b, (aggressive && t == rounds - 1) ? 1 : 0);
        enqueue_iterations(ctx, b, 0, iters, count, t * kMaxIters, unique_hi);
        int rc = enqueue_read_off(ctx, b, t, t * kMaxIters + iters - 1);
        if (rc) return rc;
    }
    PALACE_HIP_TRY(hipGetLastError());
    return PALACE_OK;
}

int decomp_run_checked(palace_ctx *ctx, const DecompBufs &b, int rounds, int aggressive, bool unique_hi, int64_t comp_cap,
                       int64_t vert_cap, int64_t max_iterations, uint64_t *iterations_out)
{
    PALACE_REQUIRE(rounds >= 1 && rounds <= kMaxRounds, "round count out of range");
    constexpr int kBatch = 16;
    hipLaunchKernelGGL(dec_init_kernel, wide_grid(ctx), kBlock, 0, ctx->stream, b, comp_cap, vert_cap, kBatch, 0);
    uint64_t count = 0;
    for (int t = 0; t < rounds; t++) {
        hipLaunchKernelGGL(dec_round_begin_kernel, wide_grid(ctx), kBlock, 0, ctx->stream, b, (aggressive && t == rounds - 1) ? 1 : 0);
        for (int first = 0;; first += kBatch) {
            PALACE_HIP_TRY(hipMemsetAsync(b.changed, 0, kBatch * sizeof(uint32_t), ctx->stream));
            enqueue_iterations(ctx, b, first, kBatch, &count, 0, unique_hi);
            uint32_t last = 0;
            PALACE_HIP_TRY(hipMemcpyAsync(&last, b.changed + kBatch - 1, sizeof last, hipMemcpyDeviceToHost, ctx->stream));
            PALACE_HIP_TRY(hipStreamSynchronize(ctx->stream));
            if (!last) break;
            if (static_cast<int64_t>(count) > max_iterations || count + kBatch >= (1ull << 21)) {
                set_error("matching: no fixed point after %llu iterations", static_cast<unsigned long long>(count));
                return PALACE_ESTATE;
            }
        }
        PALACE_HIP_TRY(hipMemsetAsync(b.changed, 0, kBatch * sizeof(uint32_t), ctx->stream));
        int rc = enqueue_read_off(ctx, b, t, kBatch - 1);
        if (rc) return rc;
    }
    if (iterations_out) *iterations_out = count;
    return PALACE_OK;
}

int decomp_group(palace_ctx *ctx, const DecompBufs &b, DecompRun &run, int rounds, int aggressive, bool unique_hi)
{
    const int first = kFirstGroupRounds;
    const int t0 = run.next_round, t1 = std::min(rounds, t0 + (t0 == 0 ? first : kRoundsPerGroup));
    for (int t = t0; t < t1; t++) {
        const int iters = ctx->match_iters > 0 ? std::min(ctx->match_iters, kMaxIters) : (t == 0 ? kFirstRoundIters : kLaterRoundIters);
        int rc = decomp_rounds(ctx, b, t, t + 1, rounds, aggressive, iters, unique_hi, &run.count);
        if (rc) return rc;
        run.rounds++;
    }
    run.next_round = t1;
    return PALACE_OK;
}

int decomp_finish(palace_ctx *ctx, const DecompBufs &b, DecompRun &run, int rounds, int aggressive, bool unique_hi, int64_t comp_cap,
                  int64_t vert_cap, int64_t max_iterations, DecompState *h_state, const std::function<int()> &reset_left)
{
    for (;;) {
        PALACE_HIP_TRY(hipMemcpyAsync(h_state, b.st, sizeof *h_state, hipMemcpyDeviceToHost, ctx->stream));
        PALACE_HIP_TRY(hipStreamSynchronize(ctx->stream));
        if (h_state->unsettled) {
            int rc = reset_left();
            if (rc) return rc;
            run.checked = true; run.rounds = rounds; run.count = 0;
            rc = decomp_run_checked(ctx, b, rounds, aggressive, unique_hi, comp_cap, vert_cap, max_iterations, &run.count);
            if (rc) return rc;
            PALACE_HIP_TRY(hipMemcpyAsync(h_state, b.st, sizeof *h_state, hipMemcpyDeviceToHost, ctx->stream));
            PALACE_HIP_TRY(hipStreamSynchronize(ctx->stream));
            return PALACE_OK;
        }
        if (run.next_round >= rounds) return PALACE_OK;
        if (h_state->alive_after == 0) {
            if (!aggressive) return PALACE_OK;
            run.next_round = rounds - 1;
        }
        int rc = decomp_group(ctx, b, run, rounds, aggressive, unique_hi);
        if (rc) return rc;
    }
}

}
```

palace_amd/csrc/decomp.hpp:

```cpp
#pragma once
#include <functional>

#include "common.hpp"

struct palace_match_result {
    int64_t n = 0;
    int64_t *off = nullptr;
    int32_t *verts = nullptr, *iter = nullptr, *open_at = nullptr;
    uint8_t *kind = nullptr;
    uint64_t *bare = nullptr;
    int64_t n_bare = 0;
    bool borrowed = false;
    ~palace_match_result();
};

namespace palace {

constexpr int kDecompGrid = 256;
constexpr int kDecompBlock = 256;
constexpr int kMaxRounds = 1024;
constexpr int kMaxIters = 64;

struct DecompState {
    int32_t S, V;
    int64_t E;
    int64_t n_comp, n_vert;
    int64_t comp_cap, vert_cap;
    uint32_t unsettled;
    uint32_t overflow;
    uint32_t bad;
    uint32_t dead;
    uint32_t packed;
    uint64_t scan_total;
    int64_t alive_after;
};

struct DecompBufs {
    DecompState *st = nullptr;
    int32_t *src = nullptr, *dst = nullptr;
    uint64_t *khi = nullptr, *klo = nullptr;
    uint8_t *done = nullptr;
    uint64_t *kc = nullptr;
    const uint32_t *pack_bad = nullptr;
    int64_t *left = nullptr;
    int32_t *orig = nullptr;
    int32_t *next = nullptr, *prev = nullptr, *on_path = nullptr, *open_at = nullptr;
    uint64_t *nhi = nullptr, *nlo = nullptr;
    uint64_t *bo_hi = nullptr, *bi_hi = nullptr;
    uint64_t *bo_lo = nullptr, *bi_lo = nullptr;
    uint64_t *len_a = nullptr, *pos = nullptr;
    int64_t *pay = nullptr;
    uint8_t *alive = nullptr, *kind = nullptr;
    uint64_t *partials = nullptr;
    uint32_t *changed = nullptr;
    int64_t *o_off = nullptr;
    int32_t *o_verts = nullptr, *o_iter = nullptr, *o_open = nullptr;
    uint8_t *o_kind = nullptr;
};

size_t decomp_bytes(int64_t s_cap, int64_t e_cap, int64_t comp_cap, int64_t vert_cap, int rounds, int iters);
void decomp_carve(DecompBufs &b, char *base, int64_t s_cap, int64_t e_cap, int64_t comp_cap, int64_t vert_cap, int rounds, int iters);
constexpr int kFirstRoundIters = 7, kLaterRoundIters = 4, kRoundsPerGroup = 5, kFirstGroupRounds = 5;
int decomp_begin(palace_ctx *ctx, const DecompBufs &b, int rounds, int64_t comp_cap, int64_t vert_cap);
int decomp_rounds(palace_ctx *ctx, const DecompBufs &b, int t0, int t1, int rounds, int aggressive, int iters, bool unique_hi,
                  uint64_t *count);

struct DecompRun { int next_round = 0; uint64_t count = 0; int rounds = 0; bool checked = false; };
int decomp_group(palace_ctx *ctx, const DecompBufs &b, DecompRun &run, int rounds, int aggressive, bool unique_hi);
int decomp_finish(palace_ctx *ctx, const DecompBufs &b, DecompRun &run, int rounds, int aggressive, bool unique_hi, int64_t comp_cap,
                  int64_t vert_cap, int64_t max_iterations, DecompState *h_state, const std::function<int()> &reset_left);

int decomp_run_checked(palace_ctx *ctx, const DecompBufs &b, int rounds, int aggressive, bool unique_hi, int64_t comp_cap,
                       int64_t vert_cap, int64_t max_iterations, uint64_t *iterations_out = nullptr);

inline void decomp_note_run(palace_ctx *ctx, const DecompRun &run, const DecompState &h_state, bool unique_hi)
{
    ctx->match_last[0] = unique_hi ? 0 : (h_state.packed ? 2 : 1);
    ctx->match_last[1] = run.checked ? 1 : 0;
    ctx->match_last[2] = run.rounds;
    ctx->match_last[3] = static_cast<int64_t>(run.count);
}

int scan_u64(palace_ctx *ctx, const uint64_t *in, uint64_t *out, const int32_t *n_dev, uint64_t *partials, uint64_t *total_dev);

}
```

palace_amd/csrc/filter.hip:

```cpp
#include <algorithm>
#include <cstdlib>
#include <memory>
#include <vector>

#include "common.hpp"
#include "decomp.hpp"

namespace palace {
namespace {

constexpr uint64_t kEmptyKey = ~0ull;
constexpr uint64_t kWeightTop = 1ull << 40;

struct FilterState {
    int32_t n_segs, S_f, n_sel, n_resc;
    int64_t n_edges, n_junc, n_kept2, n_kept3, n_arcs;
    int64_t n_static, n_dyn;
    int64_t n_path_arcs;
    uint32_t bad, pack_bad;
    uint64_t scan_total;
};
enum : uint32_t { kBadPathToken = 1, kBadNoSeg = 2, kBadEdgeBound = 4, kBadArcTable = 8 };

struct ArcTable {
// ... 282 lines not shown
        const palace_graph_edge e = edges[i];
        const int64_t w = min(edge_total(e), static_cast<int64_t>(kWeightTop - 1));
        const int32_t cu = 2 * e.left + (e.oL & 1), cv = 2 * e.right + (e.oR & 1);
        const int32_t u = 2 * f.fid[e.left] + (e.oL & 1), v = 2 * f.fid[e.right] + (e.oR & 1);
        bump_arc(f, cu, cv, u, v, w);
        if ((v ^ 1) != u) bump_arc(f, cv ^ 1, cu ^ 1, v ^ 1, u ^ 1, w);
    }
}

__global__ void st4_arcs_dyn_kernel(F f)
{
    FilterState *fs = f.fs;
    const int64_t n_static = min(fs->n_static, f.arc_cap), n = min(fs->n_dyn, f.t.list_cap);
    for (int64_t a = gtid(); a < n; a += gsize()) {
        const int64_t s = f.t.list[a];
        const uint64_t key = f.t.key[s];
        const int64_t at = n_static + a;
        if (at < f.arc_cap) {
            f.arc_u[at] = static_cast<int32_t>(key >> 32); f.arc_v[at] = static_cast<int32_t>(key & 0xffffffffu);
            f.arc_w[at] = f.t.w[s]; f.arc_backed[at] = 0;
        } else atomicOr(&fs->bad, kBadArcTable);
        f.t.key[s] = kEmptyKey; f.t.w[s] = 0;
    }
    if (gtid() == 0) fs->n_arcs = min(n_static + n, f.arc_cap);
}

__global__ void st4_arc_keys_kernel(F f, DecompBufs b)
{
    const int64_t n = min(f.fs->n_static, f.arc_cap) + min(f.fs->n_dyn, f.t.list_cap);
    for (int64_t a = gtid(); a < n && a < f.arc_cap; a += gsize()) {
        const int32_t u = f.arc_u[a], v = f.arc_v[a];
        const uint64_t w = min(static_cast<uint64_t>(f.arc_w[a]), kWeightTop - 1);
        b.khi[a] = ((kWeightTop - w) << 1) | (f.arc_backed[a] ? 0u : 1u);
        const uint64_t key = (static_cast<uint64_t>(static_cast<uint32_t>(u)) << 32) | static_cast<uint32_t>(v);
        const uint64_t twin = (static_cast<uint64_t>(static_cast<uint32_t>(v ^ 1)) << 32) | static_cast<uint32_t>(u ^ 1);
        const uint64_t cls = min(key, twin);
        b.klo[a] = (cls << 1) | (key != cls ? 1u : 0u);
        f.has_arc[u >> 1] = 1; f.has_arc[v >> 1] = 1;
    }
}

__global__ void st4_sub_in_kernel(F f)
{
    const int n = f.fs->S_f;
    for (int i = gtid(); i < n; i += gsize()) f.scan_in[i] = f.has_arc[i];
}

__global__ void st4_sub_kernel(F f, DecompBufs b, const int32_t *__restrict__ cn)
{
    FilterState *fs = f.fs;
    const int n = fs->S_f;
    const int32_t n_sub = static_cast<int32_t>(fs->scan_total);
    for (int i = gtid(); i < n; i += gsize()) {
        if (!f.has_arc[i]) continue;
        const int32_t sub = static_cast<int32_t>(f.scan_out[i]);
        b.orig[sub] = i;
        b.left[sub] = max(1, cn[f.contig_of[i]]);
    }
    const int64_t n_arcs = min(fs->n_arcs, f.arc_cap);
    const int vbits = 32 - __clz(max(1, 2 * n_sub - 1)), wbits = min(40, 51 - 2 * vbits);
    const uint64_t wmax = wbits > 0 ? (1ull << wbits) - 1 : 0;
    if (gtid() == 0 && wbits <= 0) fs->pack_bad = 1;
    for (int64_t a = gtid(); a < n_arcs; a += gsize()) {
        const int32_t u = f.arc_u[a], v = f.arc_v[a];
        const int32_t su = 2 * static_cast<int32_t>(f.scan_out[u >> 1]) + (u & 1), sv = 2 * static_cast<int32_t>(f.scan_out[v >> 1]) + (v & 1);
        b.src[a] = su;
        b.dst[a] = sv;
        if (wbits > 0) {
            const uint64_t w = f.arc_w[a];
            if (w > wmax) atomicOr(&fs->pack_bad, 1u);
            const uint64_t key = (static_cast<uint64_t>(su) << vbits) | static_cast<uint32_t>(sv);
            const uint64_t twin = (static_cast<uint64_t>(sv ^ 1) << vbits) | static_cast<uint32_t>(su ^ 1);
            b.kc[a] = ((wmax - min(w, wmax)) << (2 * vbits + 1)) | (static_cast<uint64_t>(f.arc_backed[a] ? 0u : 1u) << (2 * vbits)) | min(key, twin);
        }
    }
    if (gtid() == 0) { b.st->S = n_sub; b.st->V = 2 * n_sub; b.st->E = n_arcs; }
}

__global__ void st4_left_kernel(F f, DecompBufs b, const int32_t *__restrict__ cn)
{
    const int n = f.fs->S_f;
    for (int i = gtid(); i < n; i += gsize())
        if (f.has_arc[i]) b.left[static_cast<int32_t>(f.scan_out[i])] = max(1, cn[f.contig_of[i]]);
}

__global__ void st4_bare_kernel(F f)
{
    const int n = f.fs->S_f, words = (n + 63) / 64;
    for (int w = gtid(); w < words; w += gsize()) {
        uint64_t bits = 0;
        for (int k = 0; k < 64 && w * 64 + k < n; k++)
            if (!f.has_arc[w * 64 + k]) bits |= 1ull << k;
        f.bare[w] = bits;
    }
}

size_t up(size_t v) { return (v + 255) / 256 * 256; }
uint64_t pow2_at_least(uint64_t v) { uint64_t p = 1024; while (p < v) p <<= 1; return p; }

template <class T>
T *carve(char *&p, size_t n)
{
    T *r = reinterpret_cast<T *>(p);
    p += up(std::max<size_t>(1, n) * sizeof(T));
    return r;
}

}
}

struct palace_stage04 {
    palace::F f{};
    palace::DecompBufs b{};
    char *fixed = nullptr;
    char *grown = nullptr;
    size_t grown_bytes = 0;
    int64_t n_tok = 0, edge_bound = 0, s_cap = 0, e_cap = 0, comp_cap = 0, vert_cap = 0;
    int rounds = 0, aggressive = 0, last_rounds = 0;
    palace::DecompRun run;
    bool filtered = false, matched = false;
    const int32_t *d_cn = nullptr;
    char *pin = nullptr;
    size_t pin_bytes = 0;
    palace::FilterState *h_fs = nullptr;
    palace::DecompState *h_ds = nullptr;
    palace_match_result res;
    int32_t *h_contig_of = nullptr;
};

using namespace palace;

namespace {

const dim3 kG(1024), kB(kDecompBlock);

int grow_pinned(palace_ctx *ctx, palace_stage04 *s, size_t bytes)
{
    if (s->pin_bytes >= bytes) return PALACE_OK;
    if (s->pin) { PALACE_HIP_TRY(hipStreamSynchronize(ctx->stream)); PALACE_HIP_TRY(hipHostFree(s->pin)); s->pin = nullptr; s->pin_bytes = 0; }
    const size_t want = bytes + bytes / 4 + (1 << 16);
    hipError_t e = hipHostMalloc(reinterpret_cast<void **>(&s->pin), want, hipHostMallocDefault);
    if (e != hipSuccess) { set_error("stage04: hipHostMalloc(%zu) failed: %s", want, hipGetErrorString(e)); return PALACE_ENOMEM; }
    s->pin_bytes = want;
    return PALACE_OK;
}

int grow_device(palace_ctx *ctx, palace_stage04 *s, int64_t edge_bound, int rounds)
{
    const int64_t e_dyn = 2 * edge_bound + 16;
    const int64_t e_cap = e_dyn + s->f.pa.n + 16;
    const int64_t s_cap = std::min<int64_t>(s->f.n_segs, e_cap);
    const int64_t comp_cap = static_cast<int64_t>(rounds) * s_cap + 16, vert_cap = 2 * comp_cap;
    const uint64_t slots = pow2_at_least(2 * static_cast<uint64_t>(e_dyn));
    const size_t dec = decomp_bytes(s_cap, e_cap, comp_cap, vert_cap, rounds, kMaxIters);
    const size_t bytes = up(static_cast<size_t>(edge_bound) + 1) + up(slots * 8) * 2 + up(static_cast<size_t>(e_dyn) * 8) +
                         2 * up(static_cast<size_t>(e_cap) * 4) + up(static_cast<size_t>(e_cap) * 8) + up(static_cast<size_t>(e_cap)) + dec + 8192;
    if (s->grown_bytes < bytes || s->edge_bound < edge_bound || s->rounds < rounds) {
        if (s->grown) { PALACE_HIP_TRY(hipStreamSynchronize(ctx->stream)); PALACE_HIP_TRY(hipFree(s->grown)); s->grown = nullptr; s->grown_bytes = 0; }
        hipError_t e = hipMalloc(reinterpret_cast<void **>(&s->grown), bytes);
        if (e != hipSuccess) { set_error("stage04: hipMalloc(%zu) failed: %s", bytes, hipGetErrorString(e)); return PALACE_ENOMEM; }
        s->grown_bytes = bytes;
        char *p = s->grown;
        s->f.edge_flags = carve<uint8_t>(p, static_cast<size_t>(edge_bound) + 1);
        s->f.t.key = carve<uint64_t>(p, slots);
        s->f.t.w = carve<unsigned long long>(p, slots);
        s->f.t.backed = nullptr;
        s->f.t.mask = slots - 1;
        s->f.t.list = carve<int64_t>(p, static_cast<size_t>(e_dyn));
        s->f.t.list_cap = e_dyn;
        s->f.arc_u = carve<int32_t>(p, static_cast<size_t>(e_cap));
        s->f.arc_v = carve<int32_t>(p, static_cast<size_t>(e_cap));
        s->f.arc_w = carve<unsigned long long>(p, static_cast<size_t>(e_cap));
        s->f.arc_backed = carve<uint8_t>(p, static_cast<size_t>(e_cap));
        s->f.arc_cap = e_cap;
        decomp_carve(s->b, p, s_cap, e_cap, comp_cap, vert_cap, rounds, kMaxIters);
        s->b.pack_bad = &s->f.fs->pack_bad;
        PALACE_HIP_TRY(hipMemsetAsync(s->f.t.key, 0xff, slots * 8, ctx->stream));
        PALACE_HIP_TRY(hipMemsetAsync(s->f.t.w, 0, slots * 8, ctx->stream));
        s->edge_bound = edge_bound; s->s_cap = s_cap; s->e_cap = e_cap; s->comp_cap = comp_cap; s->vert_cap = vert_cap; s->rounds = rounds;
    }
    s->f.edge_bound = s->edge_bound;
    return PALACE_OK;
}

}

extern "C" {

int palace_stage04_create(palace_ctx *ctx, const palace_stage04_inputs *in, palace_stage04 **out)
{
    PALACE_REQUIRE(ctx && in && out, "null argument");
    PALACE_REQUIRE(in->n_segs >= 0 && in->n_segs < (1 << 30) && in->n_paths >= 0 && in->min_count >= 0, "bad size");
    PALACE_REQUIRE(in->n_segs == 0 || (in->seed && in->tlen && in->rank && in->name_len), "null per-contig array");
    PALACE_REQUIRE(in->n_paths == 0 || (in->path_off && in->path_tok), "null path arrays");
    PALACE_HIP_TRY(hipSetDevice(ctx->device));
    const size_t n = static_cast<size_t>(in->n_segs);
    const int64_t n_tok = in->n_paths ? in->path_off[in->n_paths] : 0;
    PALACE_REQUIRE(n_tok >= 0 && (in->n_paths == 0 || in->path_off[0] == 0), "path offsets must start at 0 and ascend");
    int64_t n_pairs = 0;
    for (int64_t k = 0; k < in->n_paths; k++) {
        const int64_t len = in->path_off[k + 1] - in->path_off[k];
        PALACE_REQUIRE(len >= 0 && in->path_off[k + 1] <= n_tok, "path offsets must start at 0 and ascend");
        n_pairs += len > 1 ? len - 1 : 0;
    }
    for (int32_t i = 0; i < in->n_segs; i++) PALACE_REQUIRE(in->rank[i] >= 0 && in->rank[i] < in->n_segs, "rank out of range");
    for (int64_t k = 0; k < n_tok; k++) PALACE_REQUIRE(in->path_tok[k] < 2 * static_cast<int64_t>(in->n_segs), "path token out of range");
    std::unique_ptr<palace_stage04> s(new palace_stage04());
    const int64_t pa_cap = 2 * n_pairs + 16;
    const uint64_t pa_slots = pow2_at_least(2 * static_cast<uint64_t>(pa_cap));
    const size_t bytes = up(sizeof(FilterState)) + up(n) * 8 + up(n * 4) * 6 + up(n * 8) * 2 + up((static_cast<size_t>(in->n_paths) + 1) * 8) +
                         up(static_cast<size_t>(n_tok) * 4 + 4) + up((n + 63) / 64 * 8 + 8) + up(pa_slots * 8) + up(pa_slots * 4) +
                         3 * up(static_cast<size_t>(pa_cap) * 4) + 16384;
    hipError_t e = hipMalloc(reinterpret_cast<void **>(&s->fixed), bytes);
    if (e != hipSuccess) { set_error("stage04: hipMalloc(%zu) failed: %s", bytes, hipGetErrorString(e)); return PALACE_ENOMEM; }
    char *p = s->fixed;
    F &f = s->f;
    f.fs = carve<FilterState>(p, 1);
    f.n_segs = in->n_segs; f.min_count = in->min_count; f.n_paths = in->n_paths;
    uint8_t *seed = carve<uint8_t>(p, n);
    f.core = carve<uint8_t>(p, n); f.sel = carve<uint8_t>(p, n); f.near = carve<uint8_t>(p, n); f.resc = carve<uint8_t>(p, n);
    f.seg_flags = carve<uint8_t>(p, n); f.has_arc = carve<uint8_t>(p, n);
    int32_t *tlen = carve<int32_t>(p, n), *rank = carve<int32_t>(p, n), *name_len = carve<int32_t>(p, n);
    f.by_rank = carve<int32_t>(p, n); f.fid = carve<int32_t>(p, n); f.contig_of = carve<int32_t>(p, n);
    f.scan_in = carve<uint64_t>(p, n); f.scan_out = carve<uint64_t>(p, n);
    int64_t *path_off = carve<int64_t>(p, static_cast<size_t>(in->n_paths) + 1);
    int32_t *path_tok = carve<int32_t>(p, static_cast<size_t>(n_tok) + 1);
    f.bare = carve<uint64_t>(p, (n + 63) / 64 + 1);
    f.pa.key = carve<uint64_t>(p, pa_slots); f.pa.idx = carve<int32_t>(p, pa_slots); f.pa.mask = pa_slots - 1;
    f.pa.u = carve<int32_t>(p, static_cast<size_t>(pa_cap)); f.pa.v = carve<int32_t>(p, static_cast<size_t>(pa_cap));
    f.pa.arc_of = carve<int32_t>(p, static_cast<size_t>(pa_cap));
    f.pa.cap = pa_cap; f.pa.n = 0;
    f.seed = seed; f.tlen = tlen; f.rank = rank; f.name_len = name_len; f.path_off = path_off; f.path_tok = path_tok;
    s->n_tok = n_tok;
    auto fail = [&](hipError_t err) {
        set_error("stage04: upload failed: %s", hipGetErrorString(err));
        (void)hipFree(s->fixed);
        return PALACE_EHIP;
    };
    hipStream_t st = ctx->stream;
    if (n) {
        if ((e = hipMemcpyAsync(seed, in->seed, n, hipMemcpyHostToDevice, st)) != hipSuccess) return fail(e);
        if ((e = hipMemcpyAsync(tlen, in->tlen, n * 4, hipMemcpyHostToDevice, st)) != hipSuccess) return fail(e);
        if ((e = hipMemcpyAsync(rank, in->rank, n * 4, hipMemcpyHostToDevice, st)) != hipSuccess) return fail(e);
        if ((e = hipMemcpyAsync(name_len, in->name_len, n * 4, hipMemcpyHostToDevice, st)) != hipSuccess) return fail(e);
    }
    if (in->n_paths) {
        if ((e = hipMemcpyAsync(path_off, in->path_off, (static_cast<size_t>(in->n_paths) + 1) * 8, hipMemcpyHostToDevice, st)) != hipSuccess) return fail(e);
        if (n_tok && (e = hipMemcpyAsync(path_tok, in->path_tok, static_cast<size_t>(n_tok) * 4, hipMemcpyHostToDevice, st)) != hipSuccess) return fail(e);
    } else if ((e = hipMemsetAsync(path_off, 0, 8, st)) != hipSuccess) return fail(e);
    hipLaunchKernelGGL(st4_by_rank_kernel, kG, kB, 0, st, f);
    if ((e = hipMemsetAsync(f.fs, 0, sizeof(FilterState), st)) != hipSuccess) return fail(e);
    if ((e = hipMemsetAsync(f.pa.key, 0xff, pa_slots * 8, st)) != hipSuccess) return fail(e);
    hipLaunchKernelGGL(st4_path_arcs_kernel, kG, kB, 0, st, f);
    FilterState h_fs{};
    if ((e = hipMemcpyAsync(&h_fs, f.fs, sizeof h_fs, hipMemcpyDeviceToHost, st)) != hipSuccess) return fail(e);
    if ((e = hipStreamSynchronize(st)) != hipSuccess) return fail(e);
    if (h_fs.n_path_arcs > pa_cap) { (void)hipFree(s->fixed); set_error("stage04: path arc table too small"); return PALACE_ESTATE; }
    f.pa.n = h_fs.n_path_arcs;
    e = hipHostMalloc(reinterpret_cast<void **>(&s->h_fs), up(sizeof(FilterState)) + up(sizeof(DecompState)), hipHostMallocDefault);
    if (e != hipSuccess) { (void)hipFree(s->fixed); set_error("stage04: hipHostMalloc failed: %s", hipGetErrorString(e)); return PALACE_ENOMEM; }
    s->h_ds = reinterpret_cast<DecompState *>(reinterpret_cast<char *>(s->h_fs) + up(sizeof(FilterState)));
    s->res.borrowed = true;
    *out = s.release();
    return PALACE_OK;
}

int palace_stage04_destroy(palace_ctx *ctx, palace_stage04 *s)
{
    if (!s) return PALACE_OK;
    if (ctx) { (void)hipSetDevice(ctx->device); (void)hipStreamSynchronize(ctx->stream); }
    if (s->fixed) (void)hipFree(s->fixed);
    if (s->grown) (void)hipFree(s->grown);
    if (s->pin) (void)hipHostFree(s->pin);
    if (s->h_fs) (void)hipHostFree(s->h_fs);
    delete s;
    return PALACE_OK;
}

int palace_stage04_reserve(palace_ctx *ctx, palace_stage04 *s, int64_t edge_bound)
{
    PALACE_REQUIRE(ctx && s && edge_bound >= 0, "bad argument");
    PALACE_HIP_TRY(hipSetDevice(ctx->device));
    return grow_device(ctx, s, std::max<int64_t>(edge_bound, s->edge_bound), std::max(s->rounds, 11));
}

int palace_stage04_filter(palace_ctx *ctx, palace_stage04 *s, const palace_graph_edge *d_edges, const int64_t *d_n_edges,
                          int64_t edge_bound)
{
    PALACE_REQUIRE(ctx && s && d_n_edges && edge_bound >= 0, "bad argument");
    PALACE_REQUIRE(edge_bound == 0 || d_edges, "null edge array");
    PALACE_HIP_TRY(hipSetDevice(ctx->device));
    int rc = grow_device(ctx, s, std::max<int64_t>(edge_bound, s->edge_bound), std::max(s->rounds, 11));
    if (rc) return rc;
    rc = [&]() -> int {
        const F &f = s->f;
        hipStream_t st = ctx->stream;
        hipLaunchKernelGGL(st4_begin_kernel, kG, kB, 0, st, f, d_n_edges, edge_bound);
        hipLaunchKernelGGL(st4_pass2_kernel, kG, kB, 0, st, f, d_edges);
        hipLaunchKernelGGL(st4_pass3_kernel, kG, kB, 0, st, f, d_edges);
        hipLaunchKernelGGL(st4_paths_kernel, kG, kB, 0, st, f);
        hipLaunchKernelGGL(st4_order_kernel, kG, kB, 0, st, f);
        PALACE_HIP_TRY(hipGetLastError());
        int rc2 = scan_u64(ctx, f.scan_in, f.scan_out, &f.fs->n_segs, s->b.partials, &f.fs->scan_total);
        if (rc2) return rc2;
        hipLaunchKernelGGL(st4_ids_kernel, kG, kB, 0, st, f);
        PALACE_HIP_TRY(hipGetLastError());
        return PALACE_OK;
    }();
    if (rc) return rc;
    s->filtered = true;
    s->matched = false;
    return PALACE_OK;
}

static int enqueue_match(palace_ctx *ctx, palace_stage04 *s, const palace_graph_edge *d_edges, bool use_paths)
{
    s->f.use_paths = use_paths ? 1 : 0;
    const F &f = s->f;
    hipStream_t st = ctx->stream;
    if (use_paths) hipLaunchKernelGGL(st4_arcs_static_kernel, kG, kB, 0, st, f);
    hipLaunchKernelGGL(st4_arcs_juncs_kernel, kG, kB, 0, st, f, d_edges);
    hipLaunchKernelGGL(st4_arcs_dyn_kernel, kG, kB, 0, st, f);
    hipLaunchKernelGGL(st4_arc_keys_kernel, kG, kB, 0, st, f, s->b);
    hipLaunchKernelGGL(st4_sub_in_kernel, kG, kB, 0, st, f);
    PALACE_HIP_TRY(hipGetLastError());
    int rc = scan_u64(ctx, f.scan_in, f.scan_out, &f.fs->S_f, s->b.partials, &f.fs->scan_total);
    if (rc) return rc;
    hipLaunchKernelGGL(st4_sub_kernel, kG, kB, 0, st, f, s->b, s->d_cn);
    hipLaunchKernelGGL(st4_bare_kernel, kG, kB, 0, st, f);
    PALACE_HIP_TRY(hipGetLastError());
    return PALACE_OK;
}

int palace_stage04_match(palace_ctx *ctx, palace_stage04 *s, const palace_graph_edge *d_edges, const int32_t *d_cn,
                         int32_t iterations, int32_t aggressive, int32_t use_paths)
{
    PALACE_REQUIRE(ctx && s && d_cn && iterations >= 1, "bad argument");
    PALACE_REQUIRE(s->filtered, "palace_stage04_filter has not run");
    const int rounds = iterations + (aggressive ? 1 : 0);
    PALACE_REQUIRE(rounds <= kMaxRounds, "too many iterations");
    PALACE_REQUIRE(rounds <= s->rounds, "more rounds than the filter call reserved room for (at most 10 iterations + aggressive)");
    PALACE_HIP_TRY(hipSetDevice(ctx->device));
    s->d_cn = d_cn; s->aggressive = aggressive ? 1 : 0;
    s->f.use_paths = use_paths ? 1 : 0;
    int rc = enqueue_match(ctx, s, d_edges, use_paths != 0);
    if (rc) return rc;
    s->run = DecompRun{};
    if ((rc = decomp_begin(ctx, s->b, rounds, s->comp_cap, s->vert_cap))) return rc;
    if ((rc = decomp_group(ctx, s->b, s->run, rounds, s->aggressive, false))) return rc;
    PALACE_HIP_TRY(hipMemcpyAsync(s->h_fs, s->f.fs, sizeof(FilterState), hipMemcpyDeviceToHost, ctx->stream));
    s->rounds = std::max(s->rounds, rounds);
    s->matched = true;
    s->last_rounds = rounds;
    return PALACE_OK;
}

static int check_filter_state(const FilterState &fs)
{
    if (fs.bad & kBadPathToken) { set_error("stage04: contigs.paths names an unknown contig id (filter_graph.py:138 raises)"); return PALACE_EINVAL; }
    if (fs.bad & kBadNoSeg) { set_error("stage04: contigs.paths rescues a contig without SEG line (filter_graph.py:257 raises)"); return PALACE_EINVAL; }
    if (fs.bad & kBadEdgeBound) { set_error("stage04: more edges on the device than the bound given to palace_stage04_filter"); return PALACE_EINVAL; }
    if (fs.bad & kBadArcTable) { set_error("stage04: arc table full"); return PALACE_ESTATE; }
    return PALACE_OK;
}

int palace_stage04_counts(palace_ctx *ctx, palace_stage04 *s, int64_t counts[8])
{
    PALACE_REQUIRE(ctx && s && counts && s->filtered, "bad argument");
    PALACE_HIP_TRY(hipMemcpyAsync(s->h_fs, s->f.fs, sizeof(FilterState), hipMemcpyDeviceToHost, ctx->stream));
    PALACE_HIP_TRY(hipStreamSynchronize(ctx->stream));
    const FilterState &fs = *s->h_fs;
    int rc = check_filter_state(fs);
    if (rc) return rc;
    counts[0] = fs.n_edges; counts[1] = fs.n_junc; counts[2] = fs.n_kept2; counts[3] = fs.n_kept3;
    counts[4] = fs.n_sel; counts[5] = fs.n_resc; counts[6] = s->matched ? fs.n_arcs : -1; counts[7] = fs.S_f;
    return PALACE_OK;
}

int palace_stage04_flags(palace_ctx *ctx, palace_stage04 *s, uint8_t *h_seg_flags, uint8_t *h_edge_flags, int64_t n_edges)
{
    PALACE_REQUIRE(ctx && s && s->filtered && n_edges >= 0 && n_edges <= s->edge_bound, "bad argument");
    if (h_seg_flags && s->f.n_segs)
        PALACE_HIP_TRY(hipMemcpyAsync(h_seg_flags, s->f.seg_flags, static_cast<size_t>(s->f.n_segs), hipMemcpyDeviceToHost, ctx->stream));
    if (h_edge_flags && n_edges)
        PALACE_HIP_TRY(hipMemcpyAsync(h_edge_flags, s->f.edge_flags, static_cast<size_t>(n_edges), hipMemcpyDeviceToHost, ctx->stream));
    PALACE_HIP_TRY(hipStreamSynchronize(ctx->stream));
    return PALACE_OK;
}

int palace_stage04_result(palace_ctx *ctx, palace_stage04 *s, palace_match_result **out, const int32_t **contig_of_out,
                          int64_t *n_segs_filtered_out)
{
    PALACE_REQUIRE(ctx && s && out, "null argument");
    PALACE_REQUIRE(s->matched, "palace_stage04_match has not run");
    PALACE_HIP_TRY(hipSetDevice(ctx->device));
    hipStream_t st = ctx->stream;
    const int rounds = s->last_rounds;
    auto reset_left = [&]() -> int {
        hipLaunchKernelGGL(st4_left_kernel, kG, kB, 0, st, s->f, s->b, s->d_cn);
        PALACE_HIP_TRY(hipGetLastError());
        return PALACE_OK;
    };
    int rc = decomp_finish(ctx, s->b, s->run, rounds, s->aggressive, false, s->comp_cap, s->vert_cap, 2 * s->e_cap + 64, s->h_ds, reset_left);
    if (rc) return rc;
    decomp_note_run(ctx, s->run, *s->h_ds, false);
    rc = check_filter_state(*s->h_fs);
    if (rc) return rc;
    const DecompState &ds = *s->h_ds;
    if (ds.overflow || ds.n_comp > s->comp_cap || ds.n_vert > s->vert_cap) { set_error("stage04: component arrays too small"); return PALACE_ESTATE; }
    const size_t nc = static_cast<size_t>(ds.n_comp), nv = static_cast<size_t>(ds.n_vert), sf = static_cast<size_t>(s->h_fs->S_f);
    const size_t words = (sf + 63) / 64;
    rc = grow_pinned(ctx, s, up((nc + 1) * 8) + up(nv * 4 + 4) + 2 * up(nc * 4 + 4) + up(nc + 1) + up(words * 8 + 8) + up(sf * 4 + 4));
    if (rc) return rc;
    char *p = s->pin;
    palace_match_result &r = s->res;
    r.off = carve<int64_t>(p, nc + 1); r.verts = carve<int32_t>(p, nv + 1); r.iter = carve<int32_t>(p, nc + 1);
    r.open_at = carve<int32_t>(p, nc + 1); r.kind = carve<uint8_t>(p, nc + 1); r.bare = carve<uint64_t>(p, words + 1);
    s->h_contig_of = carve<int32_t>(p, sf + 1);
    PALACE_HIP_TRY(hipMemcpyAsync(r.off, s->b.o_off, (nc + 1) * 8, hipMemcpyDeviceToHost, st));
    if (nv) PALACE_HIP_TRY(hipMemcpyAsync(r.verts, s->b.o_verts, nv * 4, hipMemcpyDeviceToHost, st));
    if (nc) {
        PALACE_HIP_TRY(hipMemcpyAsync(r.iter, s->b.o_iter, nc * 4, hipMemcpyDeviceToHost, st));
        PALACE_HIP_TRY(hipMemcpyAsync(r.open_at, s->b.o_open, nc * 4, hipMemcpyDeviceToHost, st));
        PALACE_HIP_TRY(hipMemcpyAsync(r.kind, s->b.o_kind, nc, hipMemcpyDeviceToHost, st));
    }
    if (words) PALACE_HIP_TRY(hipMemcpyAsync(r.bare, s->f.bare, words * 8, hipMemcpyDeviceToHost, st));
    if (sf) PALACE_HIP_TRY(hipMemcpyAsync(s->h_contig_of, s->f.contig_of, sf * 4, hipMemcpyDeviceToHost, st));
    PALACE_HIP_TRY(hipStreamSynchronize(st));
    r.n = static_cast<int64_t>(nc);
    r.n_bare = static_cast<int64_t>(sf) - ds.S;
    *out = &s->res;
    if (contig_of_out) *contig_of_out = s->h_contig_of;
    if (n_segs_filtered_out) *n_segs_filtered_out = static_cast<int64_t>(sf);
    return PALACE_OK;
}

}
```

palace_amd/csrc/match.hip:

```cpp
#include "common.hpp"
#include "decomp.hpp"
#include <algorithm>
#include <map>
#include <memory>
#include <mutex>
#include <numeric>
#include <thread>

namespace palace {

constexpr int32_t kNone = -1;

struct MatchArgs {
    int32_t n_vertices;
    int64_t n_arcs;
    const int32_t *src, *dst;
    const int64_t *out_off, *in_off;
    const int32_t *out_arcs, *in_arcs;
    const uint8_t *alive;
    int32_t *next, *prev, *next_arc, *want_out, *want_in;
    unsigned int *changed;
};

__global__ void match_propose_kernel(MatchArgs a)
// ... 14 lines not shown
            }
    }
    a.want_out[v] = wo;
    a.want_in[v] = wi;
}

__global__ void match_commit_kernel(MatchArgs a)
{
    int32_t v = blockIdx.x * blockDim.x + threadIdx.x;
    if (v >= a.n_vertices) return;
    int32_t e = a.want_out[v];
    if (e == kNone) return;
    int32_t h = a.dst[e];
    if (a.want_in[h] != e) return;
    a.next[v] = h;
    a.prev[h] = v;
    a.next_arc[v] = e;
    *a.changed = 1u;
}

__global__ void match_init_kernel(MatchArgs a)
{
    int32_t v = blockIdx.x * blockDim.x + threadIdx.x;
    if (v >= a.n_vertices) return;
    a.next[v] = kNone; a.prev[v] = kNone; a.next_arc[v] = kNone;
}

}

using namespace palace;

constexpr int kRoundsPerCheck = 4;

static int enqueue_rounds(palace_ctx *ctx, const MatchArgs &a, int n)
{
    const unsigned blocks = static_cast<unsigned>((a.n_vertices + 255) / 256);
    PALACE_HIP_TRY(hipMemsetAsync(a.changed, 0, 4, ctx->stream));
    for (int k = 0; k < n; k++) {
        hipLaunchKernelGGL(match_propose_kernel, dim3(blocks), dim3(256), 0, ctx->stream, a);
        hipLaunchKernelGGL(match_commit_kernel, dim3(blocks), dim3(256), 0, ctx->stream, a);
    }
    PALACE_HIP_TRY(hipGetLastError());
    return PALACE_OK;
}

extern "C" int palace_match_greedy(palace_ctx *ctx, int32_t n_vertices, int64_t n_arcs, const int32_t *d_src,
                                   const int32_t *d_dst, const int64_t *d_out_off, const int32_t *d_out_arcs,
                                   const int64_t *d_in_off, const int32_t *d_in_arcs, const uint8_t *d_alive,
                                   int32_t *d_next, int32_t *d_prev, int32_t *d_next_arc, int32_t *rounds_out)
{
    PALACE_REQUIRE(ctx && n_vertices >= 0 && n_arcs >= 0, "bad argument");
    if (rounds_out) *rounds_out = 0;
    if (n_vertices == 0) return PALACE_OK;
    PALACE_REQUIRE(d_out_off && d_in_off && d_alive && d_next && d_prev && d_next_arc, "null device pointer");
    PALACE_REQUIRE(n_arcs == 0 || (d_src && d_dst && d_out_arcs && d_in_arcs), "null arc arrays");
    PALACE_REQUIRE(n_arcs < (1ll << 31), "arc ids must fit in int32");
    PALACE_HIP_TRY(hipSetDevice(ctx->device));
    int rc = ensure_workspace(ctx, static_cast<size_t>(n_vertices) * 8 + 256);
    if (rc) return rc;
    MatchArgs a{};
    a.n_vertices = n_vertices; a.n_arcs = n_arcs; a.src = d_src; a.dst = d_dst;
    a.out_off = d_out_off; a.in_off = d_in_off; a.out_arcs = d_out_arcs; a.in_arcs = d_in_arcs;
    a.alive = d_alive; a.next = d_next; a.prev = d_prev; a.next_arc = d_next_arc;
    a.want_out = static_cast<int32_t *>(ctx->ws.ptr);
    a.want_in = a.want_out + n_vertices;
    a.changed = reinterpret_cast<unsigned int *>(ctx->d_small);
    const unsigned blocks = static_cast<unsigned>((n_vertices + 255) / 256);
    hipLaunchKernelGGL(match_init_kernel, dim3(blocks), dim3(256), 0, ctx->stream, a);
    int rounds = 0;
    for (;;) {
        unsigned int changed = 0;
        rc = enqueue_rounds(ctx, a, kRoundsPerCheck);
        if (rc) return rc;
        PALACE_HIP_TRY(hipMemcpyAsync(&changed, ctx->d_small, 4, hipMemcpyDeviceToHost, ctx->stream));
        PALACE_HIP_TRY(hipStreamSynchronize(ctx->stream));
        rounds += kRoundsPerCheck;
        if (!changed) break;
        if (rounds > n_vertices + 2 + kRoundsPerCheck) { set_error("palace_match_greedy: no fixed point"); return PALACE_ESTATE; }
    }
    if (rounds_out) *rounds_out = rounds;
    return PALACE_OK;
}

struct SubResult {
    std::vector<int64_t> off{0};
    std::vector<int32_t> verts, iter, open_at;
    std::vector<uint8_t> kind;
};

namespace palace {

class BlockPool {
public:
    void *take(size_t bytes)
    {
        bytes = std::max<size_t>(bytes, 64);
        {
            std::lock_guard<std::mutex> g(mu_);
            for (size_t i = 0; i < free_.size(); i++)
                if (free_[i].second >= bytes && free_[i].second <= 2 * bytes + (1 << 20)) {
                    void *p = free_[i].first;
                    sizes_[p] = free_[i].second;
                    free_.erase(free_.begin() + i);
                    return p;
                }
        }
        void *p = std::malloc(bytes);
        if (p) { std::lock_guard<std::mutex> g(mu_); sizes_[p] = bytes; }
        return p;
    }
    void give(void *p)
    {
        if (!p) return;
        std::lock_guard<std::mutex> g(mu_);
        const size_t bytes = sizes_[p];
        sizes_.erase(p);
        if (free_.size() < 16) free_.emplace_back(p, bytes);
        else std::free(p);
    }

private:
    std::mutex mu_;
    std::vector<std::pair<void *, size_t>> free_;
    std::map<void *, size_t> sizes_;
};
static BlockPool g_result_pool;

struct MatchScratch {
    std::vector<int32_t> new_id, old_id, ssrc, sdst;
    std::vector<int64_t> sub_copies;
    std::vector<uint64_t> has_arc;
    SubResult sub;
};
void free_match_scratch(MatchScratch *m) { delete m; }

template <class T>
struct Borrowed {
    T &home;
    T v;
    explicit Borrowed(T &h) : home(h), v(std::move(h)) {}
    ~Borrowed() { home = std::move(v); }
    Borrowed(const Borrowed &) = delete;
    Borrowed &operator=(const Borrowed &) = delete;
};

__global__ void iota_keys_kernel(uint64_t *__restrict__ khi, uint64_t *__restrict__ klo, int64_t n)
{
    for (int64_t i = static_cast<int64_t>(blockIdx.x) * blockDim.x + threadIdx.x; i < n; i += static_cast<int64_t>(gridDim.x) * blockDim.x) {
        khi[i] = static_cast<uint64_t>(i);
        klo[i] = 0;
    }
}

}

palace_match_result::~palace_match_result()
{
    if (borrowed) return;
    for (void *p : {(void *)off, (void *)verts, (void *)iter, (void *)open_at, (void *)kind, (void *)bare}) palace::g_result_pool.give(p);
}

static int decompose_core(palace_ctx *ctx, int32_t n_segs, const int64_t *copies, const int32_t *orig, int64_t n_arcs,
                          const int32_t *src, const int32_t *dst, int32_t iterations, int32_t aggressive, SubResult *res)
{
    using namespace palace;
    const int64_t S = n_segs, E = n_arcs;
    const int rounds = iterations + (aggressive ? 1 : 0);
    PALACE_REQUIRE(rounds <= kMaxRounds, "too many iterations");
    int64_t live_rounds = 0;
    for (int64_t s = 0; s < S; s++) live_rounds += std::min<int64_t>(iterations, std::max<int64_t>(1, copies[s]));
    if (aggressive) live_rounds += S;
    const int64_t comp_cap = live_rounds, vert_cap = 2 * live_rounds;
    const size_t dev_bytes = decomp_bytes(S, E, comp_cap, vert_cap, rounds, kMaxIters);
    int rc = ensure_workspace(ctx, dev_bytes);
    if (rc) return rc;
    DecompBufs b;
    decomp_carve(b, static_cast<char *>(ctx->ws.ptr), S, E, comp_cap, vert_cap, rounds, kMaxIters);
    const size_t e4 = (static_cast<size_t>(E) * 4 + 255) / 256 * 256, s8 = (static_cast<size_t>(S) * 8 + 255) / 256 * 256,
                 s4 = (static_cast<size_t>(S) * 4 + 255) / 256 * 256;
    rc = ensure_pinned(ctx, 2 * e4 + s8 + s4 + 512);
    if (rc) return rc;
    char *pin = static_cast<char *>(ctx->pin.ptr);
    int32_t *p_src = reinterpret_cast<int32_t *>(pin), *p_dst = reinterpret_cast<int32_t *>(pin + e4);
    int64_t *p_left = reinterpret_cast<int64_t *>(pin + 2 * e4);
    int32_t *p_orig = reinterpret_cast<int32_t *>(pin + 2 * e4 + s8);
    DecompState *p_st = reinterpret_cast<DecompState *>(pin + 2 * e4 + s8 + s4);
    DecompState *p_back = p_st + 1;
    std::copy(src, src + E, p_src); std::copy(dst, dst + E, p_dst);
    for (int64_t s = 0; s < S; s++) p_left[s] = std::max<int64_t>(1, copies[s]);
    std::copy(orig, orig + S, p_orig);
    std::memset(p_st, 0, sizeof *p_st);
    p_st->S = n_segs; p_st->V = 2 * n_segs; p_st->E = E;
    hipStream_t st = ctx->stream;
    auto upload = [&]() -> int {
        PALACE_HIP_TRY(hipMemcpyAsync(b.st, p_st, sizeof *p_st, hipMemcpyHostToDevice, st));
        if (E) {
            PALACE_HIP_TRY(hipMemcpyAsync(b.src, p_src, static_cast<size_t>(E) * 4, hipMemcpyHostToDevice, st));
            PALACE_HIP_TRY(hipMemcpyAsync(b.dst, p_dst, static_cast<size_t>(E) * 4, hipMemcpyHostToDevice, st));
            hipLaunchKernelGGL(iota_keys_kernel, dim3(kDecompGrid), dim3(kDecompBlock), 0, st, b.khi, b.klo, E);
        }
        PALACE_HIP_TRY(hipMemcpyAsync(b.left, p_left, static_cast<size_t>(S) * 8, hipMemcpyHostToDevice, st));
        PALACE_HIP_TRY(hipMemcpyAsync(b.orig, p_orig, static_cast<size_t>(S) * 4, hipMemcpyHostToDevice, st));
        return PALACE_OK;
    };
    auto fail = [&](int code) { (void)hipStreamSynchronize(st); return code; };
    hipError_t e = hipSuccess;
    if ((rc = upload())) return fail(rc);
    if ((rc = decomp_begin(ctx, b, rounds, comp_cap, vert_cap))) return fail(rc);
    DecompRun run;
    if ((rc = decomp_group(ctx, b, run, rounds, aggressive, true))) return fail(rc);
    auto reset_left = [&]() -> int {
        PALACE_HIP_TRY(hipMemcpyAsync(b.left, p_left, static_cast<size_t>(S) * 8, hipMemcpyHostToDevice, st));
        return PALACE_OK;
    };
    if ((rc = decomp_finish(ctx, b, run, rounds, aggressive, true, comp_cap, vert_cap, 2 * E + 64, p_back, reset_left))) return fail(rc);
    decomp_note_run(ctx, run, *p_back, true);
    if (p_back->overflow || p_back->n_comp > comp_cap || p_back->n_vert > vert_cap) {
        set_error("decompose: component arrays too small (%lld components, %lld vertices)", (long long)p_back->n_comp, (long long)p_back->n_vert);
        return PALACE_ESTATE;
    }
    const size_t nc = static_cast<size_t>(p_back->n_comp), nv = static_cast<size_t>(p_back->n_vert);
    res->off.resize(nc + 1); res->verts.resize(nv); res->iter.resize(nc); res->open_at.resize(nc); res->kind.resize(nc);
    e = hipMemcpyAsync(res->off.data(), b.o_off, (nc + 1) * 8, hipMemcpyDeviceToHost, st);
    if (e == hipSuccess && nv) e = hipMemcpyAsync(res->verts.data(), b.o_verts, nv * 4, hipMemcpyDeviceToHost, st);
    if (e == hipSuccess && nc) e = hipMemcpyAsync(res->iter.data(), b.o_iter, nc * 4, hipMemcpyDeviceToHost, st);
    if (e == hipSuccess && nc) e = hipMemcpyAsync(res->open_at.data(), b.o_open, nc * 4, hipMemcpyDeviceToHost, st);
    if (e == hipSuccess && nc) e = hipMemcpyAsync(res->kind.data(), b.o_kind, nc, hipMemcpyDeviceToHost, st);
    if (e == hipSuccess) e = hipStreamSynchronize(st);
    if (e != hipSuccess) { set_error("decompose: %s", hipGetErrorString(e)); return fail(PALACE_EHIP); }
    return PALACE_OK;
}

namespace {

void radix_by(const std::vector<uint64_t> &key, std::vector<uint32_t> &perm, std::vector<uint32_t> &tmp)
{
    const size_t n = perm.size();
    uint64_t all_or = 0, all_and = ~0ull;
    for (size_t i = 0; i < n; i++) { all_or |= key[i]; all_and &= key[i]; }
    const uint64_t varying = all_or ^ all_and;
    std::vector<uint32_t> hist(65536);
    for (int shift = 0; shift < 64; shift += 16) {
        if (((varying >> shift) & 0xffffu) == 0) continue;
        std::fill(hist.begin(), hist.end(), 0u);
        for (size_t i = 0; i < n; i++) hist[(key[perm[i]] >> shift) & 0xffffu]++;
        uint32_t run = 0;
        for (auto &h : hist) { const uint32_t c = h; h = run; run += c; }
        for (size_t i = 0; i < n; i++) tmp[hist[(key[perm[i]] >> shift) & 0xffffu]++] = perm[i];
        perm.swap(tmp);
    }
}

}

extern "C" {

int palace_match_arcs_from_edges(const int32_t *cn, int32_t n_segs, const palace_graph_edge *edges, int64_t n_edges,
                                 int32_t min_count, int64_t *copies, int32_t *src, int32_t *dst, int64_t *weight,
                                 int64_t *n_arcs_out)
{
    PALACE_REQUIRE(n_segs >= 0 && n_edges >= 0 && n_arcs_out, "bad argument");
    PALACE_REQUIRE(n_segs == 0 || (cn && copies), "null segment arrays");
    PALACE_REQUIRE(n_edges == 0 || (edges && src && dst && weight), "null edge arrays");
    PALACE_REQUIRE(n_segs < (1 << 30) && n_edges < (1ll << 30), "graph too large for int32 ids");
    for (int32_t s = 0; s < n_segs; s++) copies[s] = std::max(1, cn[s]);
    const uint64_t V = 2ull * static_cast<uint64_t>(n_segs);
    static thread_local std::vector<uint64_t> pair, m_pair, m_cls, m_wkey;
    static thread_local std::vector<int64_t> w, m_w;
    static thread_local std::vector<uint32_t> perm, tmp;
    pair.clear(); w.clear(); m_pair.clear(); m_w.clear();
    pair.reserve(2 * n_edges); w.reserve(2 * n_edges);
    for (int64_t e = 0; e < n_edges; e++) {
        const palace_graph_edge &x = edges[e];
        const int64_t tot = static_cast<int64_t>(x.counts[0]) + x.counts[1] + x.counts[2] + x.counts[3];
        if (tot < min_count) continue;
        PALACE_REQUIRE(x.left >= 0 && x.left < n_segs && x.right >= 0 && x.right < n_segs, "edge endpoint out of range");
        const uint64_t u = 2ull * x.left + (x.oL & 1), v = 2ull * x.right + (x.oR & 1);
        pair.push_back(u * V + v); w.push_back(tot);
        if ((v ^ 1) != u) { pair.push_back((v ^ 1) * V + (u ^ 1)); w.push_back(tot); }
    }
    const size_t n = pair.size();
    perm.resize(n); tmp.resize(n);
    std::iota(perm.begin(), perm.end(), 0u);
    radix_by(pair, perm, tmp);
    m_pair.reserve(n); m_w.reserve(n);
    for (size_t i = 0; i < n; i++) {
        if (!m_pair.empty() && m_pair.back() == pair[perm[i]]) m_w.back() += w[perm[i]];
        else { m_pair.push_back(pair[perm[i]]); m_w.push_back(w[perm[i]]); }
    }
    const size_t m = m_pair.size();
    int64_t w_max = 0;
    for (int64_t x : m_w) w_max = std::max(w_max, x);
    m_cls.resize(m); m_wkey.resize(m);
    for (size_t i = 0; i < m; i++) {
        const uint64_t u = m_pair[i] / V, v = m_pair[i] % V;
        m_cls[i] = std::min(m_pair[i], (v ^ 1) * V + (u ^ 1));
        m_wkey[i] = static_cast<uint64_t>(w_max - m_w[i]);
    }
    perm.resize(m); tmp.resize(m);
    std::iota(perm.begin(), perm.end(), 0u);
    radix_by(m_cls, perm, tmp);
    radix_by(m_wkey, perm, tmp);
    for (size_t i = 0; i < m; i++) {
        const uint64_t p = m_pair[perm[i]];
        src[i] = static_cast<int32_t>(p / V); dst[i] = static_cast<int32_t>(p % V); weight[i] = m_w[perm[i]];
    }
    *n_arcs_out = static_cast<int64_t>(m);
    return PALACE_OK;
}

int palace_match_set_option(palace_ctx *ctx, const char *name, int64_t value)
{
    PALACE_REQUIRE(ctx && name, "null argument");
    if (!std::strcmp(name, "iters_per_round")) {
        PALACE_REQUIRE(value >= 0 && value <= palace::kMaxIters, "iters_per_round out of range");
        ctx->match_iters = static_cast<int>(value);
    } else if (!std::strcmp(name, "one_word_keys")) {
        PALACE_REQUIRE(value == 0 || value == 1, "one_word_keys must be 0 or 1");
        ctx->match_two_word_keys = value == 0;
    } else if (!std::strcmp(name, "decomp_grid")) {
        PALACE_REQUIRE(value >= 0 && value <= 65536, "decomp_grid out of range");
        ctx->match_grid = static_cast<int>(value);
    } else {
        palace::set_error("palace_match_set_option: unknown option '%s'", name);
        return PALACE_EINVAL;
    }
    return PALACE_OK;
}

int palace_match_last_run(palace_ctx *ctx, int64_t info[4])
{
    PALACE_REQUIRE(ctx && info, "null argument");
    PALACE_REQUIRE(ctx->match_last[0] >= 0, "no decomposition has run on the device through this context");
    std::copy(ctx->match_last, ctx->match_last + 4, info);
    return PALACE_OK;
}

int palace_match_decompose(palace_ctx *ctx, int32_t n_segs, const int64_t *copies, int64_t n_arcs,
                           const int32_t *src, const int32_t *dst, int32_t iterations, int32_t aggressive,
                           palace_match_result **out)
{
    return palace_match_decompose_ex(ctx, n_segs, copies, n_arcs, src, dst, iterations, aggressive, 0, out);
}

int palace_match_decompose_ex(palace_ctx *ctx, int32_t n_segs, const int64_t *copies, int64_t n_arcs,
                              const int32_t *src, const int32_t *dst, int32_t iterations, int32_t aggressive,
                              int32_t compact, palace_match_result **out)
{
    PALACE_REQUIRE(ctx && out && n_segs >= 0 && n_arcs >= 0 && iterations >= 1, "bad argument");
    PALACE_REQUIRE(n_segs == 0 || copies, "null copies");
    PALACE_REQUIRE(n_arcs == 0 || (src && dst), "null arc arrays");
    PALACE_REQUIRE(n_segs < (1 << 30) && n_arcs < (1ll << 31), "graph too large for int32 ids");
    PALACE_HIP_TRY(hipSetDevice(ctx->device));
    const int32_t V = 2 * n_segs;
    for (int64_t e = 0; e < n_arcs; e++)
        PALACE_REQUIRE(src[e] >= 0 && src[e] < V && dst[e] >= 0 && dst[e] < V, "arc endpoint out of range");
    if (!ctx->match_scratch) ctx->match_scratch = new palace::MatchScratch();
    palace::MatchScratch &ms = *ctx->match_scratch;
    palace::Borrowed<std::vector<int32_t>> b_new(ms.new_id), b_old(ms.old_id), b_ssrc(ms.ssrc), b_sdst(ms.sdst);
    palace::Borrowed<std::vector<int64_t>> b_sc(ms.sub_copies);
    auto &new_id = b_new.v, &old_id = b_old.v, &ssrc = b_ssrc.v, &sdst = b_sdst.v;
    auto &sub_copies = b_sc.v;
    SubResult &sub = ms.sub;
    const size_t n_words = (static_cast<size_t>(n_segs) + 63) / 64;
    palace::Borrowed<std::vector<uint64_t>> b_bits(ms.has_arc);
    auto &has_arc = b_bits.v;
    has_arc.assign(n_words, 0);
    for (int64_t e = 0; e < n_arcs; e++) {
        const int32_t a = src[e] >> 1, b = dst[e] >> 1;
        has_arc[a >> 6] |= 1ull << (a & 63);
        has_arc[b >> 6] |= 1ull << (b & 63);
    }
    new_id.resize(n_words + 1);
    old_id.clear();
    for (size_t w = 0; w < n_words; w++) {
        new_id[w] = static_cast<int32_t>(old_id.size());
        for (uint64_t x = has_arc[w]; x; x &= x - 1) old_id.push_back(static_cast<int32_t>(w * 64 + __builtin_ctzll(x)));
    }
    new_id[n_words] = static_cast<int32_t>(old_id.size());
    auto is_sub = [&](int32_t sg) { return (has_arc[sg >> 6] >> (sg & 63)) & 1ull; };
    auto sub_rank = [&](int32_t sg) {
        if (sg >= n_segs) return new_id[n_words];
        return new_id[sg >> 6] + __builtin_popcountll(has_arc[sg >> 6] & ((1ull << (sg & 63)) - 1));
    };
    const int32_t n_sub = static_cast<int32_t>(old_id.size());
    sub_copies.resize(n_sub);
    for (int32_t k = 0; k < n_sub; k++) sub_copies[k] = copies[old_id[k]];
    ssrc.resize(n_arcs); sdst.resize(n_arcs);
    for (int64_t e = 0; e < n_arcs; e++) {
        ssrc[e] = 2 * sub_rank(src[e] >> 1) + (src[e] & 1);
        sdst[e] = 2 * sub_rank(dst[e] >> 1) + (dst[e] & 1);
    }
    sub.off.assign(1, 0); sub.verts.clear(); sub.iter.clear(); sub.open_at.clear(); sub.kind.clear();
    int rc = n_sub ? decompose_core(ctx, n_sub, sub_copies.data(), old_id.data(), n_arcs, ssrc.data(), sdst.data(), iterations, aggressive, &sub)
                   : PALACE_OK;
    if (rc) return rc;
    if (!n_sub) { const int64_t none[4] = {0, 0, 0, 0}; std::copy(none, none + 4, ctx->match_last); }
    const int64_t n_sub_comp = static_cast<int64_t>(sub.kind.size());
    const int last_round = iterations + (aggressive ? 1 : 0) - 1;
    const int64_t n_bare = static_cast<int64_t>(n_segs) - n_sub;
    if (compact) {
        palace_match_result *res = new palace_match_result();
        const int64_t nv = static_cast<int64_t>(sub.verts.size());
        res->off = static_cast<int64_t *>(palace::g_result_pool.take((n_sub_comp + 1) * 8));
        res->kind = static_cast<uint8_t *>(palace::g_result_pool.take(n_sub_comp + 1));
        res->iter = static_cast<int32_t *>(palace::g_result_pool.take((n_sub_comp + 1) * 4));
        res->open_at = static_cast<int32_t *>(palace::g_result_pool.take((n_sub_comp + 1) * 4));
        res->verts = static_cast<int32_t *>(palace::g_result_pool.take((nv + 1) * 4));
        res->bare = static_cast<uint64_t *>(palace::g_result_pool.take((n_words + 1) * 8));
        if (!res->off || !res->kind || !res->iter || !res->open_at || !res->verts || !res->bare) {
            delete res;
            palace::set_error("palace_match_decompose: out of host memory");
            return PALACE_ENOMEM;
        }
        std::copy(sub.off.begin(), sub.off.end(), res->off);
        std::copy(sub.kind.begin(), sub.kind.end(), res->kind);
        std::copy(sub.iter.begin(), sub.iter.end(), res->iter);
        std::copy(sub.open_at.begin(), sub.open_at.end(), res->open_at);
        std::copy(sub.verts.begin(), sub.verts.end(), res->verts);
        for (size_t w = 0; w < n_words; w++) res->bare[w] = ~has_arc[w];
        if (n_segs & 63) res->bare[n_words - 1] &= (1ull << (n_segs & 63)) - 1;
        res->n = n_sub_comp;
        res->n_bare = n_bare;
        *out = res;
        return PALACE_OK;
    }
    const int64_t n_out = n_sub_comp + n_bare * (aggressive && last_round > 0 ? 2 : 1);
    const int64_t nv_out = static_cast<int64_t>(sub.verts.size()) + (n_out - n_sub_comp);
    palace_match_result *res = new palace_match_result();
    res->off = static_cast<int64_t *>(palace::g_result_pool.take((n_out + 1) * 8));
    res->kind = static_cast<uint8_t *>(palace::g_result_pool.take(n_out));
    res->iter = static_cast<int32_t *>(palace::g_result_pool.take(n_out * 4));
    res->open_at = static_cast<int32_t *>(palace::g_result_pool.take(n_out * 4));
    res->verts = static_cast<int32_t *>(palace::g_result_pool.take(nv_out * 4));
    if (!res->off || !res->kind || !res->iter || !res->open_at || !res->verts) {
        delete res;
        palace::set_error("palace_match_decompose: out of host memory");
        return PALACE_ENOMEM;
    }
    int64_t *r_off = res->off;
    int32_t *r_verts = res->verts, *r_iter = res->iter, *r_open = res->open_at;
    uint8_t *r_kind = res->kind;
    r_off[0] = 0;
    auto split = [&](int64_t c) { return (sub.verts[sub.off[c]] + 1) >> 1; };
    auto merge_range = [&](int32_t a, int32_t b, int64_t c_lo, int64_t c_hi, int64_t oc, int64_t ov, int round) {
        int32_t s = a;
        auto bare_until = [&](int32_t until) {
            for (; s < until; s++) {
                if (is_sub(s)) continue;
                r_verts[ov++] = 2 * s;
                r_kind[oc] = 0; r_iter[oc] = round; r_open[oc] = 0;
                r_off[++oc] = ov;
            }
        };
        for (int64_t c = c_lo; c < c_hi; c++) {
            bare_until(std::min<int32_t>(b, split(c)));
            const int64_t len = sub.off[c + 1] - sub.off[c];
            std::copy(sub.verts.begin() + sub.off[c], sub.verts.begin() + sub.off[c + 1], r_verts + ov);
            ov += len;
            r_kind[oc] = sub.kind[c]; r_iter[oc] = sub.iter[c]; r_open[oc] = sub.open_at[c];
            r_off[++oc] = ov;
        }
        bare_until(b);
    };
    int64_t oc = 0, ov = 0, c = 0;
    for (int round = 0; round <= last_round; round++) {
        int64_t c_end = c;
        while (c_end < n_sub_comp && sub.iter[c_end] == round) c_end++;
        const bool bare_round = round == 0 || (aggressive && round == last_round);
        if (!bare_round) {
            merge_range(0, 0, c, c_end, oc, ov, round);
            oc += c_end - c; ov += sub.off[c_end] - sub.off[c];
            c = c_end;
            continue;
        }
        const int n_thr = n_segs >= (1 << 17) ? 4 : 1;
        std::vector<std::thread> pool;
        int64_t c_lo = c;
        for (int k = 0; k < n_thr; k++) {
            const int32_t a = static_cast<int32_t>(static_cast<int64_t>(n_segs) * k / n_thr);
            const int32_t b = static_cast<int32_t>(static_cast<int64_t>(n_segs) * (k + 1) / n_thr);
            int64_t c_hi = c_end;
            if (k + 1 < n_thr) {
                int64_t lo = c_lo, hi = c_end;
                while (lo < hi) { const int64_t mid = (lo + hi) / 2; if (split(mid) < b) lo = mid + 1; else hi = mid; }
                c_hi = lo;
            }
            const int64_t n_sub_in = sub_rank(b) - sub_rank(a);
            const int64_t n_bare_in = (b - a) - n_sub_in;
            if (n_thr == 1) merge_range(a, b, c_lo, c_hi, oc, ov, round);
            else pool.emplace_back(merge_range, a, b, c_lo, c_hi, oc, ov, round);
            oc += n_bare_in + (c_hi - c_lo);
            ov += n_bare_in + (sub.off[c_hi] - sub.off[c_lo]);
            c_lo = c_hi;
        }
        for (auto &t : pool) t.join();
        c = c_end;
    }
    res->n = oc;
    *out = res;
    return PALACE_OK;
}

int64_t palace_match_result_count(const palace_match_result *r) { return r ? r->n : 0; }
const int64_t *palace_match_result_offsets(const palace_match_result *r) { return r ? r->off : nullptr; }
const int32_t *palace_match_result_verts(const palace_match_result *r) { return r ? r->verts : nullptr; }
const uint8_t *palace_match_result_kind(const palace_match_result *r) { return r ? r->kind : nullptr; }
const int32_t *palace_match_result_iter(const palace_match_result *r) { return r ? r->iter : nullptr; }
const int32_t *palace_match_result_open_at(const palace_match_result *r) { return r ? r->open_at : nullptr; }
const uint64_t *palace_match_result_bare(const palace_match_result *r) { return r ? r->bare : nullptr; }
int64_t palace_match_result_bare_count(const palace_match_result *r) { return r ? r->n_bare : 0; }
void palace_match_result_free(palace_match_result *r) { if (r && !r->borrowed) delete r; }

}
```

Measured before the change: 112.4 million.

## Exploit reverse-complement arc symmetry to halve arc work in decomposition

Detects on the host when the arc list is closed under reverse-complement pairing, uploads only one representative arc per pair, and uses a single mirrored slot array in which a vertex's in-slot is its twin's out-slot. Commit then writes both the arc and its mirror, and keys come from each arc's original position. This is meant to cut edge-loop work, atomics and slot memory in the propose and commit kernels roughly in half. In exchange it adds a host pass to check closure and a walked-arc counter in round begin, and it relies on the key arithmetic for mirrored arcs staying consistent with the unmirrored ordering.

```diff
diff --git a/include/palace_hip.h b/include/palace_hip.h
--- a/include/palace_hip.h
+++ b/include/palace_hip.h
@@ -324,6 +324,8 @@
 typedef struct palace_match_result palace_match_result;
 int palace_match_set_option(palace_ctx *ctx, const char *name, int64_t value);
 int palace_match_last_run(palace_ctx *ctx, int64_t info[4]);
+int palace_match_last_run_ex(palace_ctx *ctx, int64_t info[8]);
+int palace_match_arcs_closed(int64_t n_arcs, const int32_t *src, const int32_t *dst, int32_t *closed_out, int64_t *n_classes_out);
 int palace_match_decompose(palace_ctx *ctx, int32_t n_segs, const int64_t *copies, int64_t n_arcs,
                            const int32_t *src, const int32_t *dst, int32_t iterations, int32_t aggressive,
                            palace_match_result **out);
diff --git a/palace_amd/capi.py b/palace_amd/capi.py
--- a/palace_amd/capi.py
+++ b/palace_amd/capi.py
@@ -178,6 +178,8 @@
                                      C.c_void_p, C.c_void_p, C.POINTER(C.c_int64)],
     "palace_match_set_option": [C.c_void_p, C.c_char_p, C.c_int64],
     "palace_match_last_run": [C.c_void_p, C.POINTER(C.c_int64)],
+    "palace_match_last_run_ex": [C.c_void_p, C.POINTER(C.c_int64)],
+    "palace_match_arcs_closed": [C.c_int64, C.POINTER(C.c_int32), C.POINTER(C.c_int32), C.POINTER(C.c_int32), C.POINTER(C.c_int64)],
     "palace_match_decompose":[C.c_void_p, C.c_int32, C.c_void_p, C.c_int64, C.c_void_p, C.c_void_p, C.c_int32,
                                C.c_int32, C.POINTER(C.c_void_p)],
     "palace_match_decompose_ex": [C.c_void_p, C.c_int32, C.c_void_p, C.c_int64, C.c_void_p, C.c_void_p, C.c_int32,
@@ -1439,6 +1441,23 @@
     return dict(key_mode=int(info[0]), checked_rerun=bool(info[1]), rounds=int(info[2]), iterations=int(info[3]))
 
 
+def match_last_run_ex(ctx: "Ctx") -> dict:
+    info = (C.c_int64 * 8)()
+    _check(lib().palace_match_last_run_ex(ctx.h, info), "palace_match_last_run_ex")
+    return dict(key_mode=int(info[0]), checked_rerun=bool(info[1]), rounds=int(info[2]), iterations=int(info[3]),
+                arcs_walked=int(info[4]), arcs=int(info[5]), mirrored=bool(info[6]))
+
+
+def match_arcs_closed(src, dst):
+    s = np.ascontiguousarray(src, dtype=np.int32)
+    d = np.ascontiguousarray(dst, dtype=np.int32)
+    assert len(s) == len(d)
+    closed, n = C.c_int32(0), C.c_int64(0)
+    _check(lib().palace_match_arcs_closed(len(s), s.ctypes.data_as(C.POINTER(C.c_int32)), d.ctypes.data_as(C.POINTER(C.c_int32)),
+                                          C.byref(closed), C.byref(n)), "palace_match_arcs_closed")
+    return bool(closed.value), int(n.value)
+
+
 def match_greedy(ctx: "Ctx", n_vertices: int, src, dst, alive=None):
     s = np.ascontiguousarray(src, dtype=np.int32)
     d = np.ascontiguousarray(dst, dtype=np.int32)
diff --git a/palace_amd/csrc/common.hpp b/palace_amd/csrc/common.hpp
--- a/palace_amd/csrc/common.hpp
+++ b/palace_amd/csrc/common.hpp
@@ -84,7 +84,7 @@
     int match_grid = 0;
     bool match_two_word_keys = false;
     int match_iters = 0;
-    int64_t match_last[4] = {-1, 0, 0, 0};
+    int64_t match_last[8] = {-1, 0, 0, 0, 0, 0, 0, 0};
     uint64_t *d_small = nullptr;
 };
 
diff --git a/palace_amd/csrc/decomp.hip b/palace_amd/csrc/decomp.hip
--- a/palace_amd/csrc/decomp.hip
+++ b/palace_amd/csrc/decomp.hip
@@ -8,6 +8,7 @@
 
 constexpr uint64_t kNoKey = ~0ull;
 constexpr uint64_t kClosed = 0;
+constexpr uint8_t kNeverWalked = 2;
 constexpr int kStampShift = 42;
 constexpr int kPackedShift = 52, kPackedStamps = 1 << (64 - kPackedShift);
 constexpr uint64_t kLenMask = (1ull << 40) - 1;
@@ -103,33 +104,63 @@
 {
     DecompState *st = b.st;
     const int V = st->V;
-    for (int i = T.tid; i < V; i += T.n) { b.bo_hi[i] = kNoKey; b.bi_hi[i] = kNoKey; b.on_path[i] = 0; }
+    for (int i = T.tid; i < V; i += T.n) b.on_path[i] = 0;
+    const bool pairs = (b.route & kRouteMirrored) && (b.route & kRoutePairs);
+    const int64_t E = st->E;
+    for (int64_t e = T.tid; e < E; e += T.n) b.done[e] = pairs && b.src[e] > (b.dst[e] ^ 1) ? kNeverWalked : 0;
     for (int i = T.tid; i < n_flags; i += T.n) b.changed[i] = 0;
     if (T.tid == 0) {
         st->n_comp = 0; st->n_vert = 0; st->comp_cap = comp_cap; st->vert_cap = vert_cap;
+        st->route = b.route; st->walked = 0;
         st->unsettled = 0; st->overflow = 0; st->bad = 0; st->dead = 0; st->scan_total = 0; st->alive_after = 0;
         st->packed = (allow_packed && b.kc && b.pack_bad && *b.pack_bad == 0) ? 1u : 0u;
         if (comp_cap >= 0) b.o_off[0] = 0;
     }
 }
 
-__device__ void ph_round_begin(const DecompBufs &b, Span T, int reset_left)
+struct Slots {
+    int V, W;
+    bool mirrored;
+    __device__ __forceinline__ Slots(const DecompState *st) : V(st->V), W((st->route & kRouteMirrored) ? st->V : 2 * st->V), mirrored(st->route & kRouteMirrored) {}
+    __device__ __forceinline__ int in(int v) const { return mirrored ? (v ^ 1) : V + v; }
+};
+
+__device__ void ph_round_begin(const DecompBufs &b, Span T, int reset_left, int count_walked)
 {
     const int V = b.st->V;
     if (!reset_left && b.st->dead) return;
     if (T.tid == 0) { b.st->alive_after = 0; if (reset_left) b.st->dead = 0; }
     const int64_t E = b.st->E;
-    for (int64_t e = T.tid; e < E; e += T.n) b.done[e] = 0;
+    const uint32_t route = b.st->route;
+    int64_t walked = 0;
+    for (int64_t e = T.tid; e < E; e += T.n) {
+        const uint8_t d = b.done[e];
+        if (d == 1) b.done[e] = 0;
+        walked += d != kNeverWalked;
+    }
+    if (count_walked) {
+        __shared__ unsigned long long wg_walked;
+        if (threadIdx.x == 0) wg_walked = 0;
+        __syncthreads();
+        if (walked) atomicAdd(&wg_walked, static_cast<unsigned long long>(walked));
+        __syncthreads();
+        if (threadIdx.x == 0 && wg_walked) atomicAdd(reinterpret_cast<unsigned long long *>(&b.st->walked), wg_walked);
+    }
     const bool packed = b.st->packed != 0;
+    const int W = (route & kRouteMirrored) ? V : 2 * V;
     for (int i = T.tid; i < V; i += T.n) {
         const int s = i >> 1;
         const int64_t l = reset_left ? 1 : b.left[s];
         if (reset_left && !(i & 1)) b.left[s] = 1;
         b.alive[i] = l > 0;
         b.next[i] = -1; b.prev[i] = -1;
-        b.bo_hi[i] = b.bi_hi[i] = l > 0 ? kNoKey : kClosed;
-        if (!packed) { b.bo_lo[i] = kNoKey; b.bo_lo[V + i] = kNoKey; b.bi_lo[i] = kNoKey; b.bi_lo[V + i] = kNoKey; }
         b.len_a[i] = 0;
+    }
+    for (int i = T.tid; i < W; i += T.n) {
+        const int v = i < V ? i : i - V;
+        const bool live = reset_left || b.left[v >> 1] > 0;
+        b.slot[i] = live ? kNoKey : kClosed;
+        if (!packed) { b.slot_lo[i] = kNoKey; b.slot_lo[W + i] = kNoKey; }
     }
 }
 
@@ -147,17 +178,17 @@
     if (b.st->dead) return;
     if (a.prev_flag >= 0 && !b.changed[a.prev_flag]) return;
     const int64_t E = b.st->E;
-    const int V = b.st->V;
-    const int other = (a.parity ^ 1) * V;
+    const Slots S(b.st);
+    const int other = (a.parity ^ 1) * S.W;
     const bool packed = b.st->packed != 0;
     for (int64_t e = T.tid; e < E; e += T.n) {
         if (b.done[e]) continue;
-        const int u = b.src[e], v = b.dst[e];
-        if (b.bi_hi[v] == kClosed) { b.done[e] = 1; continue; }
+        const int u = b.src[e], iv = S.in(b.dst[e]);
+        if (b.slot[iv] == kClosed) { b.done[e] = 1; continue; }
         const uint64_t k = packed ? (a.stamp_p | b.kc[e]) : (a.stamp | b.khi[e]);
-        if (atomicMin(reinterpret_cast<unsigned long long *>(&b.bo_hi[u]), static_cast<unsigned long long>(k)) == kClosed) { b.done[e] = 1; continue; }
-        atomicMin(reinterpret_cast<unsigned long long *>(&b.bi_hi[v]), static_cast<unsigned long long>(k));
-        if (!a.unique_hi && !packed) { b.bo_lo[other + u] = kNoKey; b.bi_lo[other + v] = kNoKey; }
+        if (atomicMin(reinterpret_cast<unsigned long long *>(&b.slot[u]), static_cast<unsigned long long>(k)) == kClosed) { b.done[e] = 1; continue; }
+        if (iv != u) atomicMin(reinterpret_cast<unsigned long long *>(&b.slot[iv]), static_cast<unsigned long long>(k));
+        if (!a.unique_hi && !packed) { b.slot_lo[other + u] = kNoKey; b.slot_lo[other + iv] = kNoKey; }
     }
 }
 
@@ -167,13 +198,14 @@
     if (a.prev_flag >= 0 && !b.changed[a.prev_flag]) return;
     if (b.st->packed) return;
     const int64_t E = b.st->E;
-    const int mine = a.parity * b.st->V;
+    const Slots S(b.st);
+    const int mine = a.parity * S.W;
     for (int64_t e = T.tid; e < E; e += T.n) {
         if (b.done[e]) continue;
-        const int u = b.src[e], v = b.dst[e];
+        const int u = b.src[e], iv = S.in(b.dst[e]);
         const uint64_t k = a.stamp | b.khi[e], lo = b.klo[e];
-        if (b.bo_hi[u] == k) atomicMin(reinterpret_cast<unsigned long long *>(&b.bo_lo[mine + u]), static_cast<unsigned long long>(lo));
-        if (b.bi_hi[v] == k) atomicMin(reinterpret_cast<unsigned long long *>(&b.bi_lo[mine + v]), static_cast<unsigned long long>(lo));
+        if (b.slot[u] == k) atomicMin(reinterpret_cast<unsigned long long *>(&b.slot_lo[mine + u]), static_cast<unsigned long long>(lo));
+        if (iv != u && b.slot[iv] == k) atomicMin(reinterpret_cast<unsigned long long *>(&b.slot_lo[mine + iv]), static_cast<unsigned long long>(lo));
     }
 }
 
@@ -188,18 +220,23 @@
 {
     bool any = false;
     const int64_t E = b.st->E;
-    const int mine = a.parity * b.st->V;
+    const Slots S(b.st);
+    const int mine = a.parity * S.W;
     const bool packed = b.st->packed != 0;
     for (int64_t e = T.tid; e < E; e += T.n) {
         if (b.done[e]) continue;
-        const int u = b.src[e], v = b.dst[e];
+        const int u = b.src[e], v = b.dst[e], iv = S.in(v);
         const uint64_t k = packed ? (a.stamp_p | b.kc[e]) : (a.stamp | b.khi[e]);
-        if (b.bo_hi[u] != k || b.bi_hi[v] != k) continue;
-        const uint64_t lo = b.klo[e];
-        if (!a.unique_hi && !packed && (b.bo_lo[mine + u] != lo || b.bi_lo[mine + v] != lo)) continue;
+        if (b.slot[u] != k || b.slot[iv] != k) continue;
+        const uint64_t hi = b.khi[e], lo = b.klo[e];
+        if (!a.unique_hi && !packed && (b.slot_lo[mine + u] != lo || b.slot_lo[mine + iv] != lo)) continue;
         b.next[u] = v; b.prev[v] = u;
-        b.nhi[u] = b.khi[e]; b.nlo[u] = lo;
-        b.bo_hi[u] = kClosed; b.bi_hi[v] = kClosed;
+        b.nhi[u] = hi; b.nlo[u] = lo;
+        if (S.mirrored && iv != u) {
+            b.next[iv] = u ^ 1; b.prev[u ^ 1] = iv;
+            b.nhi[iv] = a.unique_hi ? hi + 1 : hi; b.nlo[iv] = a.unique_hi ? lo : (lo ^ 1);
+        }
+        b.slot[u] = kClosed; b.slot[iv] = kClosed;
         b.done[e] = 1;
         any = true;
     }
@@ -296,7 +333,7 @@
 
 
 __global__ void dec_init_kernel(DecompBufs b, int64_t comp_cap, int64_t vert_cap, int n_flags, int allow_packed) { ph_init(b, whole_grid(), comp_cap, vert_cap, n_flags, allow_packed); }
-__global__ void dec_round_begin_kernel(DecompBufs b, int reset_left) { ph_round_begin(b, whole_grid(), reset_left); }
+__global__ void dec_round_begin_kernel(DecompBufs b, int reset_left, int count_walked) { ph_round_begin(b, whole_grid(), reset_left, count_walked); }
 __global__ void dec_propose_hi_kernel(DecompBufs b, IterArgs a) { ph_propose_hi(b, whole_grid(), a); }
 __global__ void dec_propose_lo_kernel(DecompBufs b, IterArgs a) { ph_propose_lo(b, whole_grid(), a); }
 __global__ void dec_commit_kernel(DecompBufs b, IterArgs a) { ph_commit(b, whole_grid(), a); }
@@ -328,7 +365,7 @@
     }
 };
 
-size_t carve_all(DecompBufs &b, char *base, int64_t s_cap, int64_t e_cap, int64_t comp_cap, int64_t vert_cap, int rounds, int iters)
+size_t carve_all(DecompBufs &b, char *base, int64_t s_cap, int64_t e_cap, int64_t comp_cap, int64_t vert_cap, int rounds, int iters, uint32_t route)
 {
     Carver c{base};
     const size_t S = static_cast<size_t>(std::max<int64_t>(1, s_cap)), V = 2 * S, E = static_cast<size_t>(std::max<int64_t>(1, e_cap));
@@ -340,8 +377,10 @@
     b.left = c.take<int64_t>(S); b.orig = c.take<int32_t>(S);
     b.next = c.take<int32_t>(V); b.prev = c.take<int32_t>(V); b.on_path = c.take<int32_t>(V); b.open_at = c.take<int32_t>(V);
     b.nhi = c.take<uint64_t>(V); b.nlo = c.take<uint64_t>(V);
-    b.bo_hi = c.take<uint64_t>(V); b.bi_hi = c.take<uint64_t>(V);
-    b.bo_lo = c.take<uint64_t>(2 * V); b.bi_lo = c.take<uint64_t>(2 * V);
+    const size_t W = (route & kRouteMirrored) ? V : 2 * V;
+    b.slot = c.take<uint64_t>(W);
+    b.slot_lo = c.take<uint64_t>(2 * W);
+    b.route = route;
     b.len_a = c.take<uint64_t>(V); b.pos = c.take<uint64_t>(V);
     b.pay = c.take<int64_t>(V);
     b.alive = c.take<uint8_t>(V); b.kind = c.take<uint8_t>(V);
@@ -357,15 +396,16 @@
 
 }
 
-size_t decomp_bytes(int64_t s_cap, int64_t e_cap, int64_t comp_cap, int64_t vert_cap, int rounds, int iters)
+size_t decomp_bytes(int64_t s_cap, int64_t e_cap, int64_t comp_cap, int64_t vert_cap, int rounds, int iters, uint32_t route)
 {
     DecompBufs tmp;
-    return carve_all(tmp, nullptr, s_cap, e_cap, comp_cap, vert_cap, rounds, iters);
-}
-
-void decomp_carve(DecompBufs &b, char *base, int64_t s_cap, int64_t e_cap, int64_t comp_cap, int64_t vert_cap, int rounds, int iters)
-{
-    carve_all(b, base, s_cap, e_cap, comp_cap, vert_cap, rounds, iters);
+    return carve_all(tmp, nullptr, s_cap, e_cap, comp_cap, vert_cap, rounds, iters, route);
+}
+
+void decomp_carve(DecompBufs &b, char *base, int64_t s_cap, int64_t e_cap, int64_t comp_cap, int64_t vert_cap, int rounds, int iters,
+                  uint32_t route)
+{
+    carve_all(b, base, s_cap, e_cap, comp_cap, vert_cap, rounds, iters, route);
 }
 
 int scan_u64(palace_ctx *ctx, const uint64_t *in, uint64_t *out, const int32_t *n_dev, uint64_t *partials, uint64_t *total_dev)
@@ -424,7 +464,7 @@
 {
     PALACE_REQUIRE(0 <= t0 && t0 <= t1 && t1 <= rounds && rounds <= kMaxRounds && iters >= 1 && iters <= kMaxIters, "round / iteration count out of range");
     for (int t = t0; t < t1; t++) {
-        hipLaunchKernelGGL(dec_round_begin_kernel, wide_grid(ctx), kBlock, 0, ctx->stream, b, (aggressive && t == rounds - 1) ? 1 : 0);
+        hipLaunchKernelGGL(dec_round_begin_kernel, wide_grid(ctx), kBlock, 0, ctx->stream, b, (aggressive && t == rounds - 1) ? 1 : 0, t == 0 ? 1 : 0);
         enqueue_iterations(ctx, b, 0, iters, count, t * kMaxIters, unique_hi);
         int rc = enqueue_read_off(ctx, b, t, t * kMaxIters + iters - 1);
         if (rc) return rc;
@@ -441,7 +481,7 @@
     hipLaunchKernelGGL(dec_init_kernel, wide_grid(ctx), kBlock, 0, ctx->stream, b, comp_cap, vert_cap, kBatch, 0);
     uint64_t count = 0;
     for (int t = 0; t < rounds; t++) {
-        hipLaunchKernelGGL(dec_round_begin_kernel, wide_grid(ctx), kBlock, 0, ctx->stream, b, (aggressive && t == rounds - 1) ? 1 : 0);
+        hipLaunchKernelGGL(dec_round_begin_kernel, wide_grid(ctx), kBlock, 0, ctx->stream, b, (aggressive && t == rounds - 1) ? 1 : 0, t == 0 ? 1 : 0);
         for (int first = 0;; first += kBatch) {
             PALACE_HIP_TRY(hipMemsetAsync(b.changed, 0, kBatch * sizeof(uint32_t), ctx->stream));
             enqueue_iterations(ctx, b, first, kBatch, &count, 0, unique_hi);
diff --git a/palace_amd/csrc/decomp.hpp b/palace_amd/csrc/decomp.hpp
--- a/palace_amd/csrc/decomp.hpp
+++ b/palace_amd/csrc/decomp.hpp
@@ -31,12 +31,17 @@
     uint32_t bad;
     uint32_t dead;
     uint32_t packed;
+    uint32_t route;
+    int64_t walked;
     uint64_t scan_total;
     int64_t alive_after;
 };
 
+constexpr uint32_t kRouteMirrored = 1, kRoutePairs = 2;
+
 struct DecompBufs {
     DecompState *st = nullptr;
+    uint32_t route = kRouteMirrored | kRoutePairs;
     int32_t *src = nullptr, *dst = nullptr;
     uint64_t *khi = nullptr, *klo = nullptr;
     uint8_t *done = nullptr;
@@ -46,8 +51,8 @@
     int32_t *orig = nullptr;
     int32_t *next = nullptr, *prev = nullptr, *on_path = nullptr, *open_at = nullptr;
     uint64_t *nhi = nullptr, *nlo = nullptr;
-    uint64_t *bo_hi = nullptr, *bi_hi = nullptr;
-    uint64_t *bo_lo = nullptr, *bi_lo = nullptr;
+    uint64_t *slot = nullptr;
+    uint64_t *slot_lo = nullptr;
     uint64_t *len_a = nullptr, *pos = nullptr;
     int64_t *pay = nullptr;
     uint8_t *alive = nullptr, *kind = nullptr;
@@ -58,8 +63,9 @@
     uint8_t *o_kind = nullptr;
 };
 
-size_t decomp_bytes(int64_t s_cap, int64_t e_cap, int64_t comp_cap, int64_t vert_cap, int rounds, int iters);
-void decomp_carve(DecompBufs &b, char *base, int64_t s_cap, int64_t e_cap, int64_t comp_cap, int64_t vert_cap, int rounds, int iters);
+size_t decomp_bytes(int64_t s_cap, int64_t e_cap, int64_t comp_cap, int64_t vert_cap, int rounds, int iters, uint32_t route);
+void decomp_carve(DecompBufs &b, char *base, int64_t s_cap, int64_t e_cap, int64_t comp_cap, int64_t vert_cap, int rounds, int iters,
+                  uint32_t route);
 constexpr int kFirstRoundIters = 7, kLaterRoundIters = 4, kRoundsPerGroup = 5, kFirstGroupRounds = 5;
 int decomp_begin(palace_ctx *ctx, const DecompBufs &b, int rounds, int64_t comp_cap, int64_t vert_cap);
 int decomp_rounds(palace_ctx *ctx, const DecompBufs &b, int t0, int t1, int rounds, int aggressive, int iters, bool unique_hi,
@@ -73,12 +79,16 @@
 int decomp_run_checked(palace_ctx *ctx, const DecompBufs &b, int rounds, int aggressive, bool unique_hi, int64_t comp_cap,
                        int64_t vert_cap, int64_t max_iterations, uint64_t *iterations_out = nullptr);
 
-inline void decomp_note_run(palace_ctx *ctx, const DecompRun &run, const DecompState &h_state, bool unique_hi)
+inline void decomp_note_run(palace_ctx *ctx, const DecompRun &run, const DecompState &h_state, bool unique_hi, int64_t graph_arcs)
 {
     ctx->match_last[0] = unique_hi ? 0 : (h_state.packed ? 2 : 1);
     ctx->match_last[1] = run.checked ? 1 : 0;
     ctx->match_last[2] = run.rounds;
     ctx->match_last[3] = static_cast<int64_t>(run.count);
+    ctx->match_last[4] = h_state.walked;
+    ctx->match_last[5] = graph_arcs;
+    ctx->match_last[6] = (h_state.route & kRouteMirrored) ? 1 : 0;
+    ctx->match_last[7] = 0;
 }
 
 int scan_u64(palace_ctx *ctx, const uint64_t *in, uint64_t *out, const int32_t *n_dev, uint64_t *partials, uint64_t *total_dev);
diff --git a/palace_amd/csrc/filter.hip b/palace_amd/csrc/filter.hip
--- a/palace_amd/csrc/filter.hip
+++ b/palace_amd/csrc/filter.hip
@@ -458,7 +458,8 @@
     const int64_t s_cap = std::min<int64_t>(s->f.n_segs, e_cap);
     const int64_t comp_cap = static_cast<int64_t>(rounds) * s_cap + 16, vert_cap = 2 * comp_cap;
     const uint64_t slots = pow2_at_least(2 * static_cast<uint64_t>(e_dyn));
-    const size_t dec = decomp_bytes(s_cap, e_cap, comp_cap, vert_cap, rounds, kMaxIters);
+    constexpr uint32_t route = kRouteMirrored | kRoutePairs;
+    const size_t dec = decomp_bytes(s_cap, e_cap, comp_cap, vert_cap, rounds, kMaxIters, route);
     const size_t bytes = up(static_cast<size_t>(edge_bound) + 1) + up(slots * 8) * 2 + up(static_cast<size_t>(e_dyn) * 8) +
                          2 * up(static_cast<size_t>(e_cap) * 4) + up(static_cast<size_t>(e_cap) * 8) + up(static_cast<size_t>(e_cap)) + dec + 8192;
     if (s->grown_bytes < bytes || s->edge_bound < edge_bound || s->rounds < rounds) {
@@ -479,7 +480,7 @@
         s->f.arc_w = carve<unsigned long long>(p, static_cast<size_t>(e_cap));
         s->f.arc_backed = carve<uint8_t>(p, static_cast<size_t>(e_cap));
         s->f.arc_cap = e_cap;
-        decomp_carve(s->b, p, s_cap, e_cap, comp_cap, vert_cap, rounds, kMaxIters);
+        decomp_carve(s->b, p, s_cap, e_cap, comp_cap, vert_cap, rounds, kMaxIters, route);
         s->b.pack_bad = &s->f.fs->pack_bad;
         PALACE_HIP_TRY(hipMemsetAsync(s->f.t.key, 0xff, slots * 8, ctx->stream));
         PALACE_HIP_TRY(hipMemsetAsync(s->f.t.w, 0, slots * 8, ctx->stream));
@@ -709,7 +710,7 @@
     };
     int rc = decomp_finish(ctx, s->b, s->run, rounds, s->aggressive, false, s->comp_cap, s->vert_cap, 2 * s->e_cap + 64, s->h_ds, reset_left);
     if (rc) return rc;
-    decomp_note_run(ctx, s->run, *s->h_ds, false);
+    decomp_note_run(ctx, s->run, *s->h_ds, false, s->h_ds->E);
     rc = check_filter_state(*s->h_fs);
     if (rc) return rc;
     const DecompState &ds = *s->h_ds;
diff --git a/palace_amd/csrc/match.hip b/palace_amd/csrc/match.hip
--- a/palace_amd/csrc/match.hip
+++ b/palace_amd/csrc/match.hip
@@ -190,6 +190,34 @@
     }
 }
 
+__global__ void position_keys_kernel(uint64_t *__restrict__ khi, uint64_t *__restrict__ klo, const int32_t *__restrict__ pos, int64_t n)
+{
+    for (int64_t i = static_cast<int64_t>(blockIdx.x) * blockDim.x + threadIdx.x; i < n; i += static_cast<int64_t>(gridDim.x) * blockDim.x) {
+        khi[i] = static_cast<uint64_t>(pos[i]);
+        klo[i] = 0;
+    }
+}
+
+bool arcs_closed(int64_t n_arcs, const int32_t *src, const int32_t *dst, int64_t *n_classes, int32_t *first_of)
+{
+    int64_t n = 0, before = -1;
+    for (int64_t i = 0; i < n_arcs;) {
+        const int32_t u = src[i], v = dst[i];
+        const bool self = v == (u ^ 1);
+        if (!self && !(i + 1 < n_arcs && src[i + 1] == (v ^ 1) && dst[i + 1] == (u ^ 1))) return false;
+        if (before >= 0) {
+            const int32_t pu = src[before], pv = dst[before];
+            if ((pu == u && pv == v) || (pu == (v ^ 1) && pv == (u ^ 1))) return false;
+        }
+        if (first_of) first_of[n] = static_cast<int32_t>(i);
+        before = i;
+        n++;
+        i += self ? 1 : 2;
+    }
+    *n_classes = n;
+    return true;
+}
+
 }
 
 palace_match_result::~palace_match_result()
@@ -209,33 +237,42 @@
     for (int64_t s = 0; s < S; s++) live_rounds += std::min<int64_t>(iterations, std::max<int64_t>(1, copies[s]));
     if (aggressive) live_rounds += S;
     const int64_t comp_cap = live_rounds, vert_cap = 2 * live_rounds;
-    const size_t dev_bytes = decomp_bytes(S, E, comp_cap, vert_cap, rounds, kMaxIters);
-    int rc = ensure_workspace(ctx, dev_bytes);
+    const size_t e4 = (static_cast<size_t>(E) * 4 + 255) / 256 * 256, s8 = (static_cast<size_t>(S) * 8 + 255) / 256 * 256,
+                 s4 = (static_cast<size_t>(S) * 4 + 255) / 256 * 256;
+    int rc = ensure_pinned(ctx, 3 * e4 + s8 + s4 + 512);
+    if (rc) return rc;
+    char *pin = static_cast<char *>(ctx->pin.ptr);
+    int32_t *p_src = reinterpret_cast<int32_t *>(pin), *p_dst = reinterpret_cast<int32_t *>(pin + e4), *p_pos = reinterpret_cast<int32_t *>(pin + 2 * e4);
+    int64_t *p_left = reinterpret_cast<int64_t *>(pin + 3 * e4);
+    int32_t *p_orig = reinterpret_cast<int32_t *>(pin + 3 * e4 + s8);
+    DecompState *p_st = reinterpret_cast<DecompState *>(pin + 3 * e4 + s8 + s4);
+    DecompState *p_back = p_st + 1;
+    int64_t n_classes = 0;
+    const bool closed = arcs_closed(E, src, dst, &n_classes, p_pos);
+    const uint32_t route = closed ? kRouteMirrored : 0;
+    const int64_t E_up = closed ? n_classes : E;
+    if (closed) for (int64_t k = 0; k < E_up; k++) { p_src[k] = src[p_pos[k]]; p_dst[k] = dst[p_pos[k]]; }
+    else { std::copy(src, src + E, p_src); std::copy(dst, dst + E, p_dst); }
+    const size_t dev_bytes = decomp_bytes(S, E_up, comp_cap, vert_cap, rounds, kMaxIters, route);
+    rc = ensure_workspace(ctx, dev_bytes);
     if (rc) return rc;
     DecompBufs b;
-    decomp_carve(b, static_cast<char *>(ctx->ws.ptr), S, E, comp_cap, vert_cap, rounds, kMaxIters);
-    const size_t e4 = (static_cast<size_t>(E) * 4 + 255) / 256 * 256, s8 = (static_cast<size_t>(S) * 8 + 255) / 256 * 256,
-                 s4 = (static_cast<size_t>(S) * 4 + 255) / 256 * 256;
-    rc = ensure_pinned(ctx, 2 * e4 + s8 + s4 + 512);
-    if (rc) return rc;
-    char *pin = static_cast<char *>(ctx->pin.ptr);
-    int32_t *p_src = reinterpret_cast<int32_t *>(pin), *p_dst = reinterpret_cast<int32_t *>(pin + e4);
-    int64_t *p_left = reinterpret_cast<int64_t *>(pin + 2 * e4);
-    int32_t *p_orig = reinterpret_cast<int32_t *>(pin + 2 * e4 + s8);
-    DecompState *p_st = reinterpret_cast<DecompState *>(pin + 2 * e4 + s8 + s4);
-    DecompState *p_back = p_st + 1;
-    std::copy(src, src + E, p_src); std::copy(dst, dst + E, p_dst);
+    decomp_carve(b, static_cast<char *>(ctx->ws.ptr), S, E_up, comp_cap, vert_cap, rounds, kMaxIters, route);
+    int32_t *d_pos = reinterpret_cast<int32_t *>(b.kc);
     for (int64_t s = 0; s < S; s++) p_left[s] = std::max<int64_t>(1, copies[s]);
     std::copy(orig, orig + S, p_orig);
     std::memset(p_st, 0, sizeof *p_st);
-    p_st->S = n_segs; p_st->V = 2 * n_segs; p_st->E = E;
+    p_st->S = n_segs; p_st->V = 2 * n_segs; p_st->E = E_up;
     hipStream_t st = ctx->stream;
     auto upload = [&]() -> int {
         PALACE_HIP_TRY(hipMemcpyAsync(b.st, p_st, sizeof *p_st, hipMemcpyHostToDevice, st));
-        if (E) {
-            PALACE_HIP_TRY(hipMemcpyAsync(b.src, p_src, static_cast<size_t>(E) * 4, hipMemcpyHostToDevice, st));
-            PALACE_HIP_TRY(hipMemcpyAsync(b.dst, p_dst, static_cast<size_t>(E) * 4, hipMemcpyHostToDevice, st));
-            hipLaunchKernelGGL(iota_keys_kernel, dim3(kDecompGrid), dim3(kDecompBlock), 0, st, b.khi, b.klo, E);
+        if (E_up) {
+            PALACE_HIP_TRY(hipMemcpyAsync(b.src, p_src, static_cast<size_t>(E_up) * 4, hipMemcpyHostToDevice, st));
+            PALACE_HIP_TRY(hipMemcpyAsync(b.dst, p_dst, static_cast<size_t>(E_up) * 4, hipMemcpyHostToDevice, st));
+            if (closed) {
+                PALACE_HIP_TRY(hipMemcpyAsync(d_pos, p_pos, static_cast<size_t>(E_up) * 4, hipMemcpyHostToDevice, st));
+                hipLaunchKernelGGL(position_keys_kernel, dim3(kDecompGrid), dim3(kDecompBlock), 0, st, b.khi, b.klo, d_pos, E_up);
+            } else hipLaunchKernelGGL(iota_keys_kernel, dim3(kDecompGrid), dim3(kDecompBlock), 0, st, b.khi, b.klo, E_up);
         }
         PALACE_HIP_TRY(hipMemcpyAsync(b.left, p_left, static_cast<size_t>(S) * 8, hipMemcpyHostToDevice, st));
         PALACE_HIP_TRY(hipMemcpyAsync(b.orig, p_orig, static_cast<size_t>(S) * 4, hipMemcpyHostToDevice, st));
@@ -252,7 +289,7 @@
         return PALACE_OK;
     };
     if ((rc = decomp_finish(ctx, b, run, rounds, aggressive, true, comp_cap, vert_cap, 2 * E + 64, p_back, reset_left))) return fail(rc);
-    decomp_note_run(ctx, run, *p_back, true);
+    decomp_note_run(ctx, run, *p_back, true, E);
     if (p_back->overflow || p_back->n_comp > comp_cap || p_back->n_vert > vert_cap) {
         set_error("decompose: component arrays too small (%lld components, %lld vertices)", (long long)p_back->n_comp, (long long)p_back->n_vert);
         return PALACE_ESTATE;
@@ -371,6 +408,23 @@
     PALACE_REQUIRE(ctx && info, "null argument");
     PALACE_REQUIRE(ctx->match_last[0] >= 0, "no decomposition has run on the device through this context");
     std::copy(ctx->match_last, ctx->match_last + 4, info);
+    return PALACE_OK;
+}
+
+int palace_match_last_run_ex(palace_ctx *ctx, int64_t info[8])
+{
+    PALACE_REQUIRE(ctx && info, "null argument");
+    PALACE_REQUIRE(ctx->match_last[0] >= 0, "no decomposition has run on the device through this context");
+    std::copy(ctx->match_last, ctx->match_last + 8, info);
+    return PALACE_OK;
+}
+
+int palace_match_arcs_closed(int64_t n_arcs, const int32_t *src, const int32_t *dst, int32_t *closed_out, int64_t *n_classes_out)
+{
+    PALACE_REQUIRE(n_arcs >= 0 && closed_out && (n_arcs == 0 || (src && dst)), "bad argument");
+    int64_t n = 0;
+    *closed_out = palace::arcs_closed(n_arcs, src, dst, &n, nullptr) ? 1 : 0;
+    if (n_classes_out) *n_classes_out = *closed_out ? n : 0;
     return PALACE_OK;
 }
 
@@ -433,7 +487,7 @@
     int rc = n_sub ? decompose_core(ctx, n_sub, sub_copies.data(), old_id.data(), n_arcs, ssrc.data(), sdst.data(), iterations, aggressive, &sub)
                    : PALACE_OK;
     if (rc) return rc;
-    if (!n_sub) { const int64_t none[4] = {0, 0, 0, 0}; std::copy(none, none + 4, ctx->match_last); }
+    if (!n_sub) { const int64_t none[8] = {0, 0, 0, 0, 0, 0, 1, 0}; std::copy(none, none + 8, ctx->match_last); }
     const int64_t n_sub_comp = static_cast<int64_t>(sub.kind.size());
     const int last_round = iterations + (aggressive ? 1 : 0) - 1;
     const int64_t n_bare = static_cast<int64_t>(n_segs) - n_sub;
```

Measured after the change: 112.9 million, median of 5. About the same (+0.4%).
